# peaceminusones/Group-GAN-GCN-GAT

Measured on AMD Instinct MI355X. Metric: scenes/sec (obs8/pred12, 20 peds) at 1/2/4/8 GPUs; ADE/FDE vs ref, higher is better.
Workload: dtype fp32; 1 GPU; train iteration = D-step + G-step (best_k=20, Adam), GAT generator; BASELINE configs[1] shape (batch 64); scenes_per_gpu=64, global_batch=64, obs_len=8, pred_len=12, generator=gat, hip_graph=True, parallelism=dp1

## Files before the change

### group-gan-gcn-gat_amd/csrc/head.hip

```cpp
#include "sgg_common.h"

namespace sgg {

namespace {

constexpr int kHeadRows = 64;

__device__ __forceinline__ float bce_grad(float x, float y) {
  const float e = expf(-fabsf(x));
  const float sg = x > 0.f ? 1.f : (x < 0.f ? -1.f : 0.f);
  return (x >= 0.f ? 1.f : 0.f) - y - sg * (e / (1.f + e));
}

template <int NT, int KT>
__global__ void __launch_bounds__(256) head_fwd_kernel(const float* __restrict__ X, int ldx, int M,
                                                       const float* __restrict__ W1, const float* __restrict__ b1,
                                                       const float* __restrict__ w2, const float* __restrict__ b2,
                                                       int act, float* __restrict__ hid, float* __restrict__ Y) {
  constexpr int K = 16 * KT, KS = 4 * KT;
  const int lane = threadIdx.x & 63, wave = threadIdx.x >> 6;
  const int c16 = lane & 15, q = lane >> 4;
  const int row0 = blockIdx.x * kHeadRows + wave * 16;
  const float* xr = X + (size_t)min(row0 + c16, M - 1) * ldx;
  float a[KS], b[KS][NT], bc[NT], wc[NT];
#pragma unroll
  for (int m = 0; m < KT; ++m) {
    const float4 xv = *reinterpret_cast<const float4*>(xr + 16 * m + 4 * q);
    a[4 * m] = xv.x;
    a[4 * m + 1] = xv.y;
    a[4 * m + 2] = xv.z;
    a[4 * m + 3] = xv.w;
#pragma unroll
    for (int t = 0; t < NT; ++t) {
      const float4 wv = *reinterpret_cast<const float4*>(W1 + (size_t)(16 * t + c16) * K + 16 * m + 4 * q);
      b[4 * m][t] = wv.x;
      b[4 * m + 1][t] = wv.y;
      b[4 * m + 2][t] = wv.z;
      b[4 * m + 3][t] = wv.w;
    }
  }
#pragma unroll
  for (int t = 0; t < NT; ++t) {
    bc[t] = b1[16 * t + c16];
    wc[t] = w2[16 * t + c16];
  }
  const float bb2 = b2[0];
  floatx4 acc[NT];
#pragma unroll
  for (int t = 0; t < NT; ++t) acc[t] = floatx4{0.f, 0.f, 0.f, 0.f};
#pragma unroll
  for (int s = 0; s < KS; ++s)
#pragma unroll
    for (int t = 0; t < NT; ++t) acc[t] = __builtin_amdgcn_mfma_f32_16x16x4f32(a[s], b[s][t], acc[t], 0, 0, 0);
  const int N1 = 16 * NT;
  float p[4] = {0.f, 0.f, 0.f, 0.f};
#pragma unroll
  for (int t = 0; t < NT; ++t)
#pragma unroll
    for (int r = 0; r < 4; ++r) {
      float h = acc[t][r] + bc[t];
      if (act & 1) h = h > 0.f ? h : 0.f;
      const int m = row0 + 4 * q + r;
      if (m < M) hid[(size_t)m * N1 + 16 * t + c16] = h;
      p[r] = fmaf(h, wc[t], p[r]);
    }
#pragma unroll
  for (int r = 0; r < 4; ++r) {
#pragma unroll
    for (int o = 1; o < 16; o <<= 1) p[r] += __shfl_xor(p[r], o);
    float y = p[r] + bb2;
    if (act & 2) y = y > 0.f ? y : 0.f;
    const int m = row0 + 4 * q + r;
    if (c16 == 0 && m < M) Y[m] = y;
  }
}

template <int NT, int KT, int DP>
__device__ __forceinline__ void head_bwd_tail(const float* __restrict__ X, int ldx, int M, int rb,
                                              const float (&dh)[kHeadRows][DP], const float (&hg)[kHeadRows][DP],
                                              const float (&g2s)[kHeadRows], const float (&wb)[4 * NT][KT],
                                              float* __restrict__ dX, int lddx, float* __restrict__ wslab) {
  constexpr int N1 = 16 * NT, K = 16 * KT;
  const int tid = threadIdx.x;
  const int lane = tid & 63, wave = tid >> 6;
  const int c16 = lane & 15, q = lane >> 4;
  {
    floatx4 acc[KT];
#pragma unroll
    for (int t = 0; t < KT; ++t) acc[t] = floatx4{0.f, 0.f, 0.f, 0.f};
#pragma unroll
    for (int s = 0; s < N1 / 4; ++s) {
      const float a = dh[16 * wave + c16][4 * s + q];
#pragma unroll
      for (int t = 0; t < KT; ++t) acc[t] = __builtin_amdgcn_mfma_f32_16x16x4f32(a, wb[s][t], acc[t], 0, 0, 0);
    }
#pragma unroll
    for (int t = 0; t < KT; ++t)
#pragma unroll
      for (int r = 0; r < 4; ++r) {
        const int m = rb + 16 * wave + 4 * q + r;
        if (m < M) dX[(size_t)m * lddx + 16 * t + c16] = acc[t][r];
      }
  }
  if (!wslab) return;
  float* row = wslab + (size_t)blockIdx.x * (N1 * K + 2 * N1 + 1);
  for (int tile = wave; tile < NT * KT; tile += 4) {
    const int mt = tile / KT, nt = tile - mt * KT;
    floatx4 acc = floatx4{0.f, 0.f, 0.f, 0.f};
    float xb[kHeadRows / 4];
#pragma unroll
    for (int s = 0; s < kHeadRows / 4; ++s)
      xb[s] = X[(size_t)min(rb + 4 * s + q, M - 1) * ldx + 16 * nt + c16];
#pragma unroll
    for (int s = 0; s < kHeadRows / 4; ++s) {
      const float a = dh[4 * s + q][16 * mt + c16];
      acc = __builtin_amdgcn_mfma_f32_16x16x4f32(a, xb[s], acc, 0, 0, 0);
    }
#pragma unroll
    for (int r = 0; r < 4; ++r) row[(size_t)(16 * mt + 4 * q + r) * K + 16 * nt + c16] = acc[r];
  }
  for (int n = tid; n < N1; n += 256) {
    float s1 = 0.f, s2 = 0.f;
    for (int r = 0; r < kHeadRows; ++r) {
      s1 += dh[r][n];
      s2 += hg[r][n];
    }
    row[N1 * K + n] = s1;
    row[N1 * K + N1 + n] = s2;
  }
  if (tid == 0) {
    float s = 0.f;
    for (int r = 0; r < kHeadRows; ++r) s += g2s[r];
    row[N1 * K + 2 * N1] = s;
  }
}

__device__ __forceinline__ float bce_dy(float y, int m, int M, float gw, float ya, float yb, int split, int nv) {
  const bool first = m < split;
  const float cnt = first ? (float)min(split, nv) : (float)min(M - split, nv);
  const bool live = first ? m < nv : m - split < nv;
  return live ? (gw / cnt) * bce_grad(y, first ? ya : yb) : 0.f;
}

template <int NT, int KT>
__global__ void __launch_bounds__(256) head_bwd_kernel(const float* __restrict__ X, int ldx, int M,
                                                       const float* __restrict__ W1, const float* __restrict__ w2,
                                                       const float* __restrict__ hid, const float* __restrict__ Y,
                                                       const float* __restrict__ dY, int act,
                                                       float* __restrict__ dX, int lddx, float* __restrict__ wslab,
                                                       const float* __restrict__ bce_g, const float* __restrict__ bce_ya,
                                                       const float* __restrict__ bce_yb, int bce_split, float bce_w,
                                                       const int32_t* __restrict__ bce_nvalid) {
  constexpr int N1 = 16 * NT, K = 16 * KT;
  constexpr int DP = N1 + 4;
  __shared__ float dh[kHeadRows][DP];
  __shared__ float hg[kHeadRows][DP];
  __shared__ float g2s[kHeadRows];
  const int tid = threadIdx.x;
  const int lane = tid & 63;
  const int c16 = lane & 15, q = lane >> 4;
  const int rb = blockIdx.x * kHeadRows;
  float wb[N1 / 4][KT];
#pragma unroll
  for (int s = 0; s < N1 / 4; ++s)
#pragma unroll
    for (int t = 0; t < KT; ++t) wb[s][t] = W1[(size_t)(4 * s + q) * K + 16 * t + c16];
  {
    constexpr int RPT = kHeadRows * N1 / 256;
    constexpr int RS = 256 / N1;
    const int n = tid % N1, r0 = tid / N1;
    const float wn = w2[n];
    float hv[RPT], yv[RPT], dyv[RPT];
#pragma unroll
    for (int i = 0; i < RPT; ++i) {
      const int mc = min(rb + r0 + RS * i, M - 1);
      hv[i] = hid[(size_t)mc * N1 + n];
      yv[i] = Y[mc];
      dyv[i] = bce_g ? 0.f : dY[mc];
    }
    if (bce_g) {
      const float gw = *bce_g * bce_w, ya = *bce_ya, yb = *bce_yb;
      const int nv = bce_nvalid ? *bce_nvalid : M;
#pragma unroll
      for (int i = 0; i < RPT; ++i) {
        const int mc = min(rb + r0 + RS * i, M - 1);
        dyv[i] = bce_dy(yv[i], mc, M, gw, ya, yb, bce_split, nv);
      }
    }
#pragma unroll
    for (int i = 0; i < RPT; ++i) {
      const int r = r0 + RS * i, m = rb + r;
      const float g = (m < M && (!(act & 2) || yv[i] > 0.f)) ? dyv[i] : 0.f;
      dh[r][n] = (!(act & 1) || hv[i] > 0.f) ? g * wn : 0.f;
      hg[r][n] = g * hv[i];
      if (n == 0) g2s[r] = g;
    }
  }
  __syncthreads();
  head_bwd_tail<NT, KT, DP>(X, ldx, M, rb, dh, hg, g2s, wb, dX, lddx, wslab);
}

template <int NT, int KT>
__global__ void __launch_bounds__(256) head_fwdbwd_kernel(
    const float* __restrict__ X, int ldx, int M, const float* __restrict__ W1, const float* __restrict__ b1,
    const float* __restrict__ w2, const float* __restrict__ b2, int act, float* __restrict__ Y,
    float* __restrict__ dX, int lddx, float* __restrict__ wslab, const float* __restrict__ bce_g,
    const float* __restrict__ bce_ya, const float* __restrict__ bce_yb, int bce_split, float bce_w,
    const int32_t* __restrict__ bce_nvalid) {
  constexpr int N1 = 16 * NT, K = 16 * KT, KS = 4 * KT;
  constexpr int DP = N1 + 4;
  __shared__ float dh[kHeadRows][DP];
  __shared__ float hg[kHeadRows][DP];
  __shared__ float g2s[kHeadRows];
  const int lane = threadIdx.x & 63, wave = threadIdx.x >> 6;
  const int c16 = lane & 15, q = lane >> 4;
  const int rb = blockIdx.x * kHeadRows;
  const int row0 = rb + wave * 16;
  const float* xr = X + (size_t)min(row0 + c16, M - 1) * ldx;
  float a[KS], b[KS][NT], bc[NT], wc[NT];
#pragma unroll
  for (int m = 0; m < KT; ++m) {
    const float4 xv = *reinterpret_cast<const float4*>(xr + 16 * m + 4 * q);
    a[4 * m] = xv.x;
    a[4 * m + 1] = xv.y;
    a[4 * m + 2] = xv.z;
    a[4 * m + 3] = xv.w;
#pragma unroll
    for (int t = 0; t < NT; ++t) {
      const float4 wv = *reinterpret_cast<const float4*>(W1 + (size_t)(16 * t + c16) * K + 16 * m + 4 * q);
      b[4 * m][t] = wv.x;
      b[4 * m + 1][t] = wv.y;
      b[4 * m + 2][t] = wv.z;
      b[4 * m + 3][t] = wv.w;
    }
  }
  float wb[N1 / 4][KT];
#pragma unroll
  for (int s = 0; s < N1 / 4; ++s)
#pragma unroll
    for (int t = 0; t < KT; ++t) wb[s][t] = W1[(size_t)(4 * s + q) * K + 16 * t + c16];
#pragma unroll
  for (int t = 0; t < NT; ++t) {
    bc[t] = b1[16 * t + c16];
    wc[t] = w2[16 * t + c16];
  }
  const float bb2 = b2[0];
  const float gw = *bce_g * bce_w, ya = *bce_ya, yb = *bce_yb;
  const int nv = bce_nvalid ? *bce_nvalid : M;
  floatx4 acc[NT];
#pragma unroll
  for (int t = 0; t < NT; ++t) acc[t] = floatx4{0.f, 0.f, 0.f, 0.f};
#pragma unroll
  for (int s = 0; s < KS; ++s)
#pragma unroll
    for (int t = 0; t < NT; ++t) acc[t] = __builtin_amdgcn_mfma_f32_16x16x4f32(a[s], b[s][t], acc[t], 0, 0, 0);
  float h[NT][4];
  float p[4] = {0.f, 0.f, 0.f, 0.f};
#pragma unroll
  for (int t = 0; t < NT; ++t)
#pragma unroll
    for (int r = 0; r < 4; ++r) {
      float v = acc[t][r] + bc[t];
      if (act & 1) v = v > 0.f ? v : 0.f;
      h[t][r] = v;
      p[r] = fmaf(v, wc[t], p[r]);
    }
#pragma unroll
  for (int r = 0; r < 4; ++r) {
#pragma unroll
    for (int o = 1; o < 16; o <<= 1) p[r] += __shfl_xor(p[r], o);
    float y = p[r] + bb2;
    if (act & 2) y = y > 0.f ? y : 0.f;
    const int lr = wave * 16 + 4 * q + r, m = rb + lr;
    if (c16 == 0 && m < M) Y[m] = y;
    const float dy = bce_dy(y, min(m, M - 1), M, gw, ya, yb, bce_split, nv);
    const float g = (m < M && (!(act & 2) || y > 0.f)) ? dy : 0.f;
#pragma unroll
    for (int t = 0; t < NT; ++t) {
      const int n = 16 * t + c16;
      dh[lr][n] = (!(act & 1) || h[t][r] > 0.f) ? g * wc[t] : 0.f;
      hg[lr][n] = g * h[t][r];
    }
    if (c16 == 0) g2s[lr] = g;
  }
  __syncthreads();
  head_bwd_tail<NT, KT, DP>(X, ldx, M, rb, dh, hg, g2s, wb, dX, lddx, wslab);
}

template <int NT>
int launch_fwd_nt(const float* X, int ldx, int M, int K, const float* W1, const float* b1, const float* w2,
                  const float* b2, int act, float* hid, float* Y, hipStream_t st) {
  const dim3 grid((M + kHeadRows - 1) / kHeadRows);
  switch (K) {
    case 16: hipLaunchKernelGGL((head_fwd_kernel<NT, 1>), grid, dim3(256), 0, st, X, ldx, M, W1, b1, w2, b2, act, hid, Y); break;
// ... 122 lines not shown
```

### group-gan-gcn-gat_amd/csrc/pool.hip

```cpp
#include <stdlib.h>
#include <string.h>

#include "sgg_common.h"
#include "pool_common.h"

namespace sgg {


constexpr int kKT = 64;
constexpr int kKTP = kKT + 2;
constexpr int kPoolWaves = 4;

struct PoolSet {
  const float* U;
  const float* pos;
  const int32_t* scene_off;
  const int4* chunks;
  int nchunks;
  const int32_t* nchunks_dev;
  float* out;
  int32_t* argmax;
};

#define SGG_POOL_PICK(s1, s2, g1)                                                       \
  const bool two_ = (int)blockIdx.x >= (g1);                                            \
  const float* __restrict__ U = two_ ? s2.U : s1.U;                                     \
  const float* __restrict__ pos = two_ ? s2.pos : s1.pos;                               \
  const int32_t* __restrict__ scene_off = two_ ? s2.scene_off : s1.scene_off;           \
  const int4* __restrict__ chunks = two_ ? s2.chunks : s1.chunks;                       \
  float* __restrict__ out = two_ ? s2.out : s1.out;                                     \
  int32_t* __restrict__ argmax = two_ ? s2.argmax : s1.argmax;                          \
  const int32_t* ncd_ = two_ ? s2.nchunks_dev : s1.nchunks_dev;                         \
  const int nch = ncd_ ? *ncd_ : (two_ ? s2.nchunks : s1.nchunks);                      \
  const int gb_ = (int)blockIdx.x - (two_ ? (g1) : 0);                                  \
  const int gstride = two_ ? (int)gridDim.x - (g1) : (g1);                              \
  const int xb = (gb_ & 7) * (gstride >> 3) + (gb_ >> 3)

template <int BN, int GPW, int UNR>
__global__ void __launch_bounds__(256)
__attribute__((amdgpu_waves_per_eu(BN == 8 && GPW == 1 ? 5 : 1))) pool_fwd_kernel(
    const PoolSet s1, const PoolSet s2, int g1, const float* __restrict__ A,
    const float* __restrict__ W2 , const float* __restrict__ b2) {
  using C = PoolCfg<BN>;
  constexpr int NT = C::NT, BNP = C::BNP;
  extern __shared__ __attribute__((aligned(16))) char smem[];
  float* Us = reinterpret_cast<float*>(smem);
  float* W2s = Us + SGG_POOL_MAX_PEDS * kKTP;
  float* As = W2s + kKT * BNP;
  float2* ps = reinterpret_cast<float2*>(As + 2 * kKT);
  unsigned long long* keys = reinterpret_cast<unsigned long long*>(ps + SGG_POOL_MAX_PEDS);
  const int lane = threadIdx.x & 63;
  const int wave = __builtin_amdgcn_readfirstlane(threadIdx.x >> 6);
  const int c16 = lane & 15, kq = lane >> 4;
  float bv[NT];
#pragma unroll
  for (int t = 0; t < NT; ++t) bv[t] = b2[min(16 * t + c16, BN - 1)];

  SGG_POOL_PICK(s1, s2, g1);
  for (int ch = xb; ch < nch; ch += gstride) {
    const int4 cd = chunks[ch];
    const int s = cd.x, i0 = cd.y, i1 = cd.z;
    if (i1 <= i0) continue;
    const int o = scene_off[s];
    const int n = scene_off[s + 1] - o;
    const int rows = i1 - i0;
    const int npairs = rows * n;

    for (int q = threadIdx.x; q < n; q += blockDim.x) ps[q] = make_float2(pos[2 * (o + q)], pos[2 * (o + q) + 1]);
    for (int q = threadIdx.x; q < rows * BN; q += blockDim.x) keys[q] = 0ull;
    __syncthreads();

    int uoff[GPW];
    float rx[GPW], ry[GPW];
    floatx4 acc[GPW][NT];
#pragma unroll
    for (int g = 0; g < GPW; ++g) {
      const int p = (wave * GPW + g) * 16 + c16;
      int il = 0, j = 0;
      if (p < npairs) { il = p / n; j = p - il * n; }
      uoff[g] = j * kKTP + kq;
      const float2 pj = ps[j], pi = ps[i0 + il];
      rx[g] = p < npairs ? pj.x - pi.x : 0.f;
      ry[g] = p < npairs ? pj.y - pi.y : 0.f;
#pragma unroll
      for (int t = 0; t < NT; ++t) acc[g][t] = floatx4{0.f, 0.f, 0.f, 0.f};
    }

    constexpr int kUQ = (SGG_POOL_MAX_PEDS * (kKT / 4) + 255) / 256;
    constexpr int kWQ = (kKT * BNP + 255) / 256;
    float4 ureg[kUQ];
    float wreg[kWQ];
    float areg = 0.f;
    auto load_tile = [&](int k0) {
#pragma unroll
      for (int e = 0; e < kUQ; ++e) {
        const int q = threadIdx.x + 256 * e;
        const int r = q / (kKT / 4), c4 = q - r * (kKT / 4);
        if (r < n) ureg[e] = *reinterpret_cast<const float4*>(U + (size_t)(o + r) * kHidden + k0 + 4 * c4);
      }
#pragma unroll
      for (int e = 0; e < kWQ; ++e) {
        const int q = threadIdx.x + 256 * e;
        const int kk = q / BNP, cc = q - kk * BNP;
        wreg[e] = (kk < kKT && cc < BN) ? W2[(size_t)cc * kHidden + k0 + kk] : 0.f;
      }
      if (threadIdx.x < 2 * kKT) areg = A[2 * k0 + threadIdx.x];
    };
    auto store_tile = [&]() {
#pragma unroll
      for (int e = 0; e < kUQ; ++e) {
        const int q = threadIdx.x + 256 * e;
        const int r = q / (kKT / 4), c4 = q - r * (kKT / 4);
        if (r < n) {
          float* d = Us + r * kKTP + 4 * c4;
          d[0] = ureg[e].x; d[1] = ureg[e].y; d[2] = ureg[e].z; d[3] = ureg[e].w;
        }
      }
#pragma unroll
      for (int e = 0; e < kWQ; ++e) {
        const int q = threadIdx.x + 256 * e;
        if (q < kKT * BNP) W2s[q] = wreg[e];
      }
      if (threadIdx.x < 2 * kKT) As[threadIdx.x] = areg;
    };
    load_tile(0);
    __syncthreads();
    store_tile();
    __syncthreads();
    for (int k0 = 0; k0 < kHidden; k0 += kKT) {
      if (k0 + kKT < kHidden) load_tile(k0 + kKT);
      float b[NT], u[GPW];
      float2 a;
#pragma unroll
      for (int t = 0; t < NT; ++t) b[t] = W2s[kq * BNP + 16 * t + c16];
      a = *reinterpret_cast<const float2*>(As + 2 * kq);
#pragma unroll
      for (int g = 0; g < GPW; ++g) u[g] = Us[uoff[g]];
#pragma unroll UNR
      for (int s4 = 0; s4 < kKT / 4; ++s4) {
        float h[GPW], bc[NT];
#pragma unroll
        for (int g = 0; g < GPW; ++g) h[g] = fmaxf(fmaf(a.y, ry[g], fmaf(a.x, rx[g], u[g])), 0.f);
#pragma unroll
        for (int t = 0; t < NT; ++t) bc[t] = b[t];
        if (s4 + 1 < kKT / 4) {
          const int kn = 4 * (s4 + 1);
#pragma unroll
          for (int t = 0; t < NT; ++t) b[t] = W2s[(kn + kq) * BNP + 16 * t + c16];
          a = *reinterpret_cast<const float2*>(As + 2 * (kn + kq));
#pragma unroll
          for (int g = 0; g < GPW; ++g) u[g] = Us[uoff[g] + kn];
        }
#pragma unroll
        for (int g = 0; g < GPW; ++g)
#pragma unroll
          for (int t = 0; t < NT; ++t) acc[g][t] = __builtin_amdgcn_mfma_f32_16x16x4f32(h[g], bc[t], acc[g][t], 0, 0, 0);
      }
// ... 681 lines not shown
    const int c = q / (kHidden / 4), c4 = q - c * (kHidden / 4);
    float4 w = make_float4(0.f, 0.f, 0.f, 0.f);
    if (c < BN) w = *reinterpret_cast<const float4*>(W2 + (size_t)c * kHidden + 4 * c4);
    __bf16* d = W2s + c * kBfWP + 4 * c4;
    d[0] = (__bf16)w.x;
    d[1] = (__bf16)w.y;
    d[2] = (__bf16)w.z;
    d[3] = (__bf16)w.w;
  }
  for (int q = tid; q < kHidden; q += kBfThreads) {
    const float2 a = reinterpret_cast<const float2*>(A)[q];
    As[q] = a.x;
    As[kHidden + q] = a.y;
  }

  SGG_POOL_PICK(s1, s2, g1);
  for (int ch = xb; ch < nch; ch += gstride) {
    const int4 cd = chunks[ch];
    const int s = cd.x;
    if (cd.z <= cd.y) continue;
    const int o = scene_off[s];
    const int n = scene_off[s + 1] - o;
    const int i0 = cd.y, R = min(cd.z - cd.y, kBfMaxRows);
    const int nj = (n + kJbRows - 1) / kJbRows;
    __syncthreads();
    for (int q = tid; q < n; q += kBfThreads) ps[q] = make_float2(pos[2 * (o + q)], pos[2 * (o + q) + 1]);
    for (int q = tid; q < R * BN; q += kBfThreads) keys[q] = 0ull;

    floatx4 ur[kJbUQ];
    auto load_block = [&](int jb) __attribute__((always_inline)) {
#pragma unroll
      for (int e = 0; e < kJbUQ; ++e) {
        const int q = tid + kBfThreads * e;
        const int row = q / (kHidden / 4), c4 = q - row * (kHidden / 4);
        const int j = jb * kJbRows + row;
        ur[e] = j < n ? *reinterpret_cast<const floatx4*>(U + (size_t)(o + j) * kHidden + 4 * c4)
                      : floatx4{0.f, 0.f, 0.f, 0.f};
      }
    };
    auto store_block = [&](int buf) __attribute__((always_inline)) {
      float* d = Uj + buf * kJbRows * kJbUP;
#pragma unroll
      for (int e = 0; e < kJbUQ; ++e) {
        const int q = tid + kBfThreads * e;
        const int row = q / (kHidden / 4), c4 = q - row * (kHidden / 4);
        *reinterpret_cast<floatx4*>(d + row * kJbUP + 4 * c4) = ur[e];
      }
    };
    load_block(0);
    store_block(0);
    if (nj > 1) load_block(1);
    __syncthreads();

    for (int jb = 0; jb < nj; ++jb) {
      const float* ut = Uj + (jb & 1) * kJbRows * kJbUP;
      const int j = jb * kJbRows + c16;
      const bool jok = j < n;
      const float2 pj = ps[jok ? j : 0];
      for (int r0 = 0; r0 < R; r0 += kBfWaves * GPW) {
        float2v rxy[GPW];
        floatx4 acc[GPW][NT];
#pragma unroll
        for (int g = 0; g < GPW; ++g) {
          const int il = r0 + wave * GPW + g;
          const float2 pi = ps[i0 + min(il, R - 1)];
          rxy[g] = jok ? float2v{pj.x - pi.x, pj.y - pi.y} : float2v{0.f, 0.f};
#pragma unroll
          for (int t = 0; t < NT; ++t) acc[g][t] = floatx4{0.f, 0.f, 0.f, 0.f};
        }
        const int ngr = min(GPW, max(0, R - r0 - wave * GPW));
        const float* urow = ut + c16 * kJbUP + 8 * kq;
#pragma unroll 2
        for (int ks = 0; ks < kHidden / 32; ++ks) {
          const int ku = 32 * ks + 8 * kq;
          float2v ax[4], ay[4];
#pragma unroll
          for (int v = 0; v < 2; ++v) {
            const float4 x = *reinterpret_cast<const float4*>(As + ku + 4 * v);
            const float4 y = *reinterpret_cast<const float4*>(As + kHidden + ku + 4 * v);
            ax[2 * v] = float2v{x.x, x.y};
            ax[2 * v + 1] = float2v{x.z, x.w};
            ay[2 * v] = float2v{y.x, y.y};
            ay[2 * v + 1] = float2v{y.z, y.w};
          }
          bf16x8_t bfr[NT];
#pragma unroll
          for (int t = 0; t < NT; ++t)
            bfr[t] = *reinterpret_cast<const bf16x8_t*>(W2s + (16 * t + c16) * kBfWP + ku);
          const float4 u0 = *reinterpret_cast<const float4*>(urow + 32 * ks);
          const float4 u1 = *reinterpret_cast<const float4*>(urow + 32 * ks + 4);
          const float2v uv[4] = {{u0.x, u0.y}, {u0.z, u0.w}, {u1.x, u1.y}, {u1.z, u1.w}};
#pragma unroll
          for (int g = 0; g < GPW; ++g) {
            if (g < ngr) {
              const float2v rx2 = rxy[g].xx, ry2 = rxy[g].yy;
              short2v hi[4];
#pragma unroll
              for (int m = 0; m < 4; ++m) {
                const float2v pre = __builtin_elementwise_fma(ay[m], ry2, __builtin_elementwise_fma(ax[m], rx2, uv[m]));
                const short2v b = __builtin_bit_cast(short2v, __builtin_convertvector(pre, bf16x2v));
                hi[m] = __builtin_elementwise_max(b, short2v{0, 0});
              }
              const short4v h01 = __builtin_shufflevector(hi[0], hi[1], 0, 1, 2, 3);
              const short4v h23 = __builtin_shufflevector(hi[2], hi[3], 0, 1, 2, 3);
              const bf16x8_t hv =
                  __builtin_bit_cast(bf16x8_t, __builtin_shufflevector(h01, h23, 0, 1, 2, 3, 4, 5, 6, 7));
#pragma unroll
              for (int t = 0; t < NT; ++t)
                acc[g][t] = __builtin_amdgcn_mfma_f32_16x16x32_bf16(hv, bfr[t], acc[g][t], 0, 0, 0);
            }
          }
        }
#pragma unroll
        for (int g = 0; g < GPW; ++g) {
          if (g < ngr) {
            const int il = r0 + wave * GPW + g;
#pragma unroll
            for (int t = 0; t < NT; ++t) {
              const int cc = 16 * t + c16;
              const float bb = cc < BN ? bv[t] : 0.f;
              unsigned long long best = 0ull;
#pragma unroll
              for (int r = 0; r < 4; ++r) {
                const int jj = jb * kJbRows + 4 * kq + r;
                float v = acc[g][t][r] + bb;
                v = v > 0.f ? v : 0.f;
                const unsigned long long key =
                    jj < n ? (((unsigned long long)__float_as_uint(v) << 32) | (0xFFFFFFFFull - (unsigned)jj)) : 0ull;
                best = umax64(best, key);
              }
              best = rows_max64(best);
              if (kq == 0 && cc < BN) atomicMax(&keys[il * BN + cc], best);
            }
          }
        }
      }
      if (jb + 1 < nj) {
        store_block((jb + 1) & 1);
        if (jb + 2 < nj) load_block(jb + 2);
      }
      __syncthreads();
    }
    for (int q = tid; q < R * BN; q += kBfThreads) {
      const unsigned long long key = keys[q];
      const size_t oi = (size_t)(o + i0) * BN + q;
      out[oi] = __uint_as_float((unsigned)(key >> 32));
      argmax[oi] = o + (int)(0xFFFFFFFFu - (unsigned)(key & 0xFFFFFFFFull));
    }
  }
}

constexpr int kBwdStageRows = 16;

template <int BN, bool WGRAD, bool STAGE>
__global__ void __launch_bounds__(512) pool_bwd_kernel(
    const float* __restrict__ U, const float* __restrict__ pos, const float* __restrict__ A,
    const float* __restrict__ W2 , const float* __restrict__ out,
    const int32_t* __restrict__ argmax, const float* __restrict__ dout, const int32_t* __restrict__ scene_off,
    int S, int jq, float* __restrict__ dU, float* __restrict__ part) {
  __shared__ unsigned long long msk[SGG_POOL_MAX_PEDS * BN];
  __shared__ float gs[SGG_POOL_MAX_PEDS * BN];
  __shared__ int jsel[SGG_POOL_MAX_PEDS * BN];
  __shared__ float2 ps[SGG_POOL_MAX_PEDS];
  extern __shared__ float Us[];
  const int k = threadIdx.x;
  float w2[BN], dw2[BN];
#pragma unroll
  for (int c = 0; c < BN; ++c) {
    w2[c] = W2[c * kHidden + k];
    dw2[c] = 0.f;
  }
  const float a0 = A[2 * k], a1 = A[2 * k + 1];
  float dA0 = 0.f, dA1 = 0.f, db2 = 0.f;
  for (int un = blockIdx.x; un < S * jq; un += gridDim.x) {
    const int s = un / jq, jp = un - s * jq;
    const int o = scene_off[s];
    const int n = scene_off[s + 1] - o;
    const int ne = n * BN;
    const int j0 = (n * jp) / jq, j1 = (n * (jp + 1)) / jq;
    if (STAGE) {
      const float* Ur = U + (size_t)(o + j0) * kHidden + k;
#pragma unroll 4
      for (int r = 0; r < j1 - j0; ++r) Us[r * kHidden + k] = Ur[(size_t)r * kHidden];
    }
#pragma unroll 2
    for (int e = k; e < ne; e += kHidden) {
      const size_t ge = (size_t)o * BN + e;
      const float ov = out[ge], dv = dout[ge];
      const int av = argmax[ge];
      gs[e] = ov > 0.f ? dv : 0.f;
      jsel[e] = av - o;
      msk[e] = 0ull;
    }
    for (int q = k; q < n; q += kHidden) ps[q] = make_float2(pos[2 * (o + q)], pos[2 * (o + q) + 1]);
    __syncthreads();
    for (int e = k; e < ne; e += kHidden) {
      if (gs[e] != 0.f) {
        const int i = e / BN, c = e - i * BN;
        atomicOr(&msk[jsel[e] * BN + c], 1ull << i);
      }
    }
    if (WGRAD && jp == 0 && k < BN)
      for (int i = 0; i < n; ++i) db2 += gs[i * BN + k];
    __syncthreads();
    const float* Uc = U + (size_t)o * kHidden + k;
    float u_next = STAGE ? 0.f : (j0 < j1 ? Uc[(size_t)j0 * kHidden] : 0.f);
    for (int j = j0; j < j1; ++j) {
      float u;
      if (STAGE) {
        u = Us[(j - j0) * kHidden + k];
      } else {
        u = u_next;
        if (j + 1 < j1) u_next = Uc[(size_t)(j + 1) * kHidden];
      }
      const float2 pj = ps[j];
      float du = 0.f;
      constexpr int CB = BN < 16 ? BN : 16;
      unsigned long long mrow[CB];
#pragma unroll
      for (int c = 0; c < BN; ++c) {
        if (c % CB == 0) {
#pragma unroll
          for (int cc = 0; cc < CB; ++cc) mrow[cc] = msk[j * BN + c + cc];
        }
        const unsigned long long mv = mrow[c % CB];
        const unsigned mhi = (unsigned)__builtin_amdgcn_readfirstlane((unsigned)(mv >> 32));
        const unsigned mlo = (unsigned)__builtin_amdgcn_readfirstlane((unsigned)mv);
        unsigned long long m = ((unsigned long long)mhi << 32) | (unsigned long long)mlo;
        auto entry = [&](float g, float2 pi) {
          const float rx = pj.x - pi.x, ry = pj.y - pi.y;
          const float pre = fmaf(a1, ry, fmaf(a0, rx, u));
          const float gm = pre > 0.f ? g : 0.f;
          const float d = gm * w2[c];
          du += d;
          if (WGRAD) {
            dw2[c] = fmaf(gm, pre, dw2[c]);
            dA0 = fmaf(d, rx, dA0);
            dA1 = fmaf(d, ry, dA1);
          }
        };
        while (m) {
          const int i = __builtin_ctzll(m);
          m &= m - 1;
          const bool two = m != 0;
          const int i2 = two ? __builtin_ctzll(m) : i;
          if (two) m &= m - 1;
          const float g = gs[i * BN + c], g2 = gs[i2 * BN + c];
          const float2 pi = ps[i], pi2 = ps[i2];
          entry(g, pi);
          if (two) entry(g2, pi2);
        }
      }
      dU[(size_t)(o + j) * kHidden + k] = du;
    }
    __syncthreads();
  }
  if (WGRAD) {
    float* row = part + (size_t)blockIdx.x * (BN * kHidden + 2 * kHidden + BN);
#pragma unroll
    for (int c = 0; c < BN; ++c) row[c * kHidden + k] = dw2[c];
    row[BN * kHidden + 2 * k] = dA0;
    row[BN * kHidden + 2 * k + 1] = dA1;
    if (k < BN) row[BN * kHidden + 2 * kHidden + k] = db2;
  }
}

template <int BN>
static size_t pool_fwd_lds(int max_rows) {
  using C = PoolCfg<BN>;
  return sizeof(float) * ((size_t)SGG_POOL_MAX_PEDS * kKTP + (size_t)kKT * C::BNP + 2 * kKT) +
         sizeof(float2) * SGG_POOL_MAX_PEDS + sizeof(unsigned long long) * (size_t)max_rows * BN;
}

static int pool_range(int nchunks) { return nchunks < 32768 ? (nchunks + 7) & ~7 : 32768; }

template <int BN, int GPW>
static void launch_fwd_g(const PoolSet& s1, const PoolSet& s2, const float* A, const float* W2, const float* b2,
                         int max_rows, int max_n, hipStream_t st) {
  const int g1 = pool_range(s1.nchunks), grid = g1 + (s2.chunks ? pool_range(s2.nchunks) : 0);
  const int nchunks = s1.nchunks + (s2.chunks ? s2.nchunks : 0);
  const size_t lds = pool_fwd_lds<BN>(max_rows);
  if constexpr (GPW <= 2 && BN >= 32 && BN <= 48) {
    const char* xe = getenv("SGG_POOL_X3");
    if (!(xe && xe[0] == '0') && max_n >= 1 && max_n <= SGG_POOL_MAX_PEDS) {
      const int umax = (max_n + 3) & ~3;
      const size_t lx = sizeof(float) * 2 * ((size_t)umax * kVP + pool_x3_tb_fixed<BN>()) +
                        sizeof(float2) * SGG_POOL_MAX_PEDS + sizeof(unsigned long long) * (size_t)max_rows * BN;
      hipLaunchKernelGGL((pool_fwd_x3_kernel<BN, GPW>), dim3(grid), dim3(256), lx, st, s1, s2, g1, A, W2, b2, umax);
      return;
    }
  }
  if constexpr (GPW <= 2) {
    const char* vv = getenv("SGG_POOL_V");
    if (nchunks <= 4 * device_cus() && !(vv && vv[0] == '0')) {
      const size_t lv = sizeof(float) * 2 * ((size_t)(SGG_POOL_MAX_PEDS + 16 * PoolCfg<BN>::NT) * kVP + 2 * kKT) +
                        sizeof(float2) * SGG_POOL_MAX_PEDS + sizeof(unsigned long long) * (size_t)max_rows * BN;
      hipLaunchKernelGGL((pool_fwd_v_kernel<BN, GPW>), dim3(grid), dim3(256), lv, st, s1, s2, g1, A, W2, b2);
      return;
    }
  }
  hipLaunchKernelGGL((pool_fwd_kernel<BN, GPW, 2>), dim3(grid), dim3(256), lds, st, s1, s2, g1, A, W2, b2);
}
static int pool_bwd_jq(int S) {
  if (S < 1) return 1;
  const int jq = 256 / S;
  return jq < 1 ? 1 : (jq > 8 ? 8 : jq);
}

template <int BN>
static int launch_fwd(const PoolSet& s1, const PoolSet& s2, const float* A, const float* W2, const float* b2,
                      int max_rows, int max_n, int gpw, hipStream_t st) {
  switch (gpw) {
    case 1: launch_fwd_g<BN, 1>(s1, s2, A, W2, b2, max_rows, max_n, st); break;
    case 2: launch_fwd_g<BN, 2>(s1, s2, A, W2, b2, max_rows, max_n, st); break;
    default: launch_fwd_g<BN, 4>(s1, s2, A, W2, b2, max_rows, max_n, st); break;
  }
  SGG_RETURN_LAUNCH("sgg_pool_fwd");
}

template <int BN>
static int launch_fwd_bf16(const PoolSet& s1, const PoolSet& s2, const float* A, const float* W2, const float* b2,
                           int gpw, int max_rows, int max_n, hipStream_t st) {
  const int n1 = s1.nchunks, n2 = s2.chunks ? s2.nchunks : 0;
  int grid = device_cus();
  if (grid > n1 + n2) grid = n1 + n2;
  grid = (grid + 7) & ~7;
  int g1 = grid;
  if (n2 > 0) {
    if (n1 == 0) {
      g1 = 0;
    } else {
      if (grid < 16) grid = 16;
      g1 = (int)(((long long)grid * n1 / (n1 + n2) + 4) & ~7LL);
      g1 = g1 < 8 ? 8 : (g1 > grid - 8 ? grid - 8 : g1);
    }
  }
  const char* jbe = getenv("SGG_POOL_JB");
  const bool jb_off = jbe && strcmp(jbe, "0") == 0;
  if (max_n >= 32 && !jb_off && pool_jb_lds_bytes<BN>() <= 160 * 1024) {
    const size_t ljb = pool_jb_lds_bytes<BN>();
#define SGG_POOL_JB(G) \
  hipLaunchKernelGGL((pool_fwd_bf16_jb_kernel<BN, G>), dim3(grid), dim3(kBfThreads), ljb, st, s1, s2, g1, A, W2, b2)
    if (max_rows > 16)
      SGG_POOL_JB(4);
    else if (max_rows > 8)
      SGG_POOL_JB(2);
    else
      SGG_POOL_JB(1);
#undef SGG_POOL_JB
    SGG_RETURN_LAUNCH("sgg_pool_fwd_bf16");
  }
  const size_t lds = pool_bf16_lds_bytes<BN>();
#define SGG_POOL_BF(G) \
  hipLaunchKernelGGL((pool_fwd_bf16_kernel<BN, G>), dim3(grid), dim3(kBfThreads), lds, st, s1, s2, g1, A, W2, b2)
  if (gpw >= 4 && BN <= 48)
    SGG_POOL_BF(4);
  else if (gpw >= 2)
    SGG_POOL_BF(2);
  else
    SGG_POOL_BF(1);
#undef SGG_POOL_BF
  SGG_RETURN_LAUNCH("sgg_pool_fwd_bf16");
}

template <int BN>
static int launch_bwd(const float* U, const float* pos, const float* A, const float* W2, const float* out,
                      const int32_t* am, const float* dout, const int32_t* off, int S, int max_n, float* dU,
                      float* part, hipStream_t st) {
  const int grid = sgg_pool_bwd_grid(S), jq = pool_bwd_jq(S);
  const int rows = (max_n + jq - 1) / jq + 1;
  const bool stage = rows <= kBwdStageRows;
  const size_t lds = stage ? sizeof(float) * (size_t)rows * kHidden : 0;
#define SGG_POOL_BWD(W, SG)                                                                                          \
  hipLaunchKernelGGL((pool_bwd_kernel<BN, W, SG>), dim3(grid), dim3(512), lds, st, U, pos, A, W2, out, am, dout, off, \
                     S, jq, dU, part)
  if (part) {
    if (stage) SGG_POOL_BWD(true, true); else SGG_POOL_BWD(true, false);
  } else {
    if (stage) SGG_POOL_BWD(false, true); else SGG_POOL_BWD(false, false);
  }
#undef SGG_POOL_BWD
  SGG_RETURN_LAUNCH("sgg_pool_bwd");
}

}

using namespace sgg;

static bool pool_bn_ok(int bn) { return bn == 8 || bn == 16 || bn == 32 || bn == 48 || bn == 64; }

static int plan_rows(int n, int gpw) {
  int rows = (16 * kPoolWaves * gpw) / n;
  if (rows > 64) rows = 64;
  return rows < 1 ? 1 : rows;
}

extern "C" int sgg_pool_plan(const int32_t* host_scene_off, int S, int bn, int target_chunks, int max_gpw,
                             int32_t* chunks, int cap, int* max_rows, int* gpw_out) {
  if (!host_scene_off || !chunks || !max_rows || !gpw_out || S < 0 || cap < 0) {
    sgg::set_error("sgg_pool_plan: bad argument");
    return SGG_E_ARG;
  }
  int gpw = bn > 16 ? 4 : 2;
  if (max_gpw > 0) {
    while (gpw > max_gpw && gpw > 1) gpw >>= 1;
  }
  for (; gpw > 1; gpw >>= 1) {
    long nc = 0;
    for (int s = 0; s < S; ++s) {
      const int n = host_scene_off[s + 1] - host_scene_off[s];
      if (n > 0) nc += (n + plan_rows(n, gpw) - 1) / plan_rows(n, gpw);
    }
    if (nc >= target_chunks) break;
  }
  int nc = 0, mr = 1;
  for (int s = 0; s < S; ++s) {
    const int n = host_scene_off[s + 1] - host_scene_off[s];
    if (n <= 0) continue;
    const int rmax = plan_rows(n, gpw), nck = (n + rmax - 1) / rmax, rows = (n + nck - 1) / nck;
    for (int i0 = 0; i0 < n; i0 += rows) {
      const int i1 = i0 + rows < n ? i0 + rows : n;
      if (nc >= cap) {
        sgg::set_error("sgg_pool_plan: chunk table capacity %d exceeded", cap);
        return SGG_E_ARG;
      }
      chunks[4 * nc + 0] = s;
      chunks[4 * nc + 1] = i0;
      chunks[4 * nc + 2] = i1;
      chunks[4 * nc + 3] = gpw;
      if (i1 - i0 > mr) mr = i1 - i0;
      ++nc;
    }
  }
  *max_rows = mr;
  *gpw_out = gpw;
  return nc;
}

extern "C" int sgg_pool_plan_bf16(const int32_t* host_scene_off, int S, int bn, int target_chunks, int32_t* chunks,
                                  int cap, int* max_rows, int* gpw_out) {
  if (!host_scene_off || !chunks || !max_rows || !gpw_out || S < 0 || cap < 0 || !pool_bn_ok(bn)) {
    sgg::set_error("sgg_pool_plan_bf16: bad argument");
    return SGG_E_ARG;
  }
  auto rows_of = [&](int n, int pb) { const int r = pb / n; return r < 1 ? 1 : (r > n ? n : r); };
  int pb = 2048;
  for (; pb > 128; pb >>= 1) {
    long nc = 0;
    for (int s = 0; s < S; ++s) {
      const int n = host_scene_off[s + 1] - host_scene_off[s];
      if (n > 0) nc += (n + rows_of(n, pb) - 1) / rows_of(n, pb);
    }
    if (nc >= target_chunks) break;
  }
  int nc = 0, mr = 1, mp = 1;
  for (int s = 0; s < S; ++s) {
    const int n = host_scene_off[s + 1] - host_scene_off[s];
    if (n <= 0) continue;
    const int rmax = rows_of(n, pb), nck = (n + rmax - 1) / rmax, rows = (n + nck - 1) / nck;
    for (int i0 = 0; i0 < n; i0 += rows) {
      const int i1 = i0 + rows < n ? i0 + rows : n;
      if (nc >= cap) {
        sgg::set_error("sgg_pool_plan_bf16: chunk table capacity %d exceeded", cap);
        return SGG_E_ARG;
      }
      chunks[4 * nc + 0] = s;
      chunks[4 * nc + 1] = i0;
      chunks[4 * nc + 2] = i1;
      chunks[4 * nc + 3] = 0;
      if (i1 - i0 > mr) mr = i1 - i0;
      if ((i1 - i0) * n > mp) mp = (i1 - i0) * n;
      ++nc;
    }
  }
  const int gmax = bn > 48 ? 2 : 4;
  int gpw = 1;
  while (gpw < gmax && 16 * kBfWaves * gpw < mp) gpw <<= 1;
  for (int c = 0; c < nc; ++c) chunks[4 * c + 3] = gpw;
  *max_rows = mr;
  *gpw_out = gpw;
  return nc;
}

static int pool_batch_check(const char* fn, const float* U, const float* pos, const int32_t* scene_off,
                            const int32_t* chunks, int nchunks, int max_rows, int gpw, int B, int max_n,
                            const float* out, const int32_t* argmax) {
  SGG_CHECK_ARG(U && pos && scene_off && chunks && out && argmax, "%s: null pointer", fn);
  SGG_CHECK_ARG(nchunks >= 0 && B >= 0, "%s: bad sizes", fn);
  SGG_CHECK_ARG(max_n >= 1 && max_n <= SGG_POOL_MAX_PEDS, "%s: max scene size %d outside [1, %d]", fn, max_n,
                SGG_POOL_MAX_PEDS);
  SGG_CHECK_ARG(max_rows >= 1 && max_rows <= 64, "%s: chunk rows %d outside [1, 64]", fn, max_rows);
  SGG_CHECK_ARG(gpw == 1 || gpw == 2 || gpw == 4, "%s: gpw %d not in {1,2,4}", fn, gpw);
  return 0;
}

static int pool_fwd_sets(const PoolSet& s1, const PoolSet& s2, const float* A, const float* W2, const float* b2,
                         int max_rows, int max_n, int gpw, int bn, bool bf16, hipStream_t st) {
  if (s1.nchunks + (s2.chunks ? s2.nchunks : 0) == 0) return 0;
  if (bf16) {
    switch (bn) {
      case 8: return launch_fwd_bf16<8>(s1, s2, A, W2, b2, gpw, max_rows, max_n, st);
      case 16: return launch_fwd_bf16<16>(s1, s2, A, W2, b2, gpw, max_rows, max_n, st);
      case 32: return launch_fwd_bf16<32>(s1, s2, A, W2, b2, gpw, max_rows, max_n, st);
      case 48: return launch_fwd_bf16<48>(s1, s2, A, W2, b2, gpw, max_rows, max_n, st);
      default: return launch_fwd_bf16<64>(s1, s2, A, W2, b2, gpw, max_rows, max_n, st);
    }
  }
  switch (bn) {
    case 8: return launch_fwd<8>(s1, s2, A, W2, b2, max_rows, max_n, gpw, st);
    case 16: return launch_fwd<16>(s1, s2, A, W2, b2, max_rows, max_n, gpw, st);
    case 32: return launch_fwd<32>(s1, s2, A, W2, b2, max_rows, max_n, gpw, st);
    case 48: return launch_fwd<48>(s1, s2, A, W2, b2, max_rows, max_n, gpw, st);
    default: return launch_fwd<64>(s1, s2, A, W2, b2, max_rows, max_n, gpw, st);
  }
}

static int pool_fwd_one(const char* fn, bool bf16, const float* U, const float* pos, const float* A, const float* W2,
                        const float* b2, const int32_t* scene_off, const int32_t* chunks, int nchunks, int max_rows,
                        int gpw, int B, int bn, int max_n, float* out, int32_t* argmax, const int32_t* nchunks_dev,
                        void* stream) {
  SGG_CHECK_ARG(A && W2 && b2, "%s: null pointer", fn);
  SGG_CHECK_ARG(pool_bn_ok(bn), "%s: bottleneck %d not built (8/16/32/48/64)", fn, bn);
  const int rc = pool_batch_check(fn, U, pos, scene_off, chunks, nchunks, max_rows, gpw, B, max_n, out, argmax);
  if (rc != 0) return rc;
  const PoolSet s1 = {U, pos, scene_off, reinterpret_cast<const int4*>(chunks), nchunks, nchunks_dev, out, argmax};
  const PoolSet none = {};
  return pool_fwd_sets(s1, none, A, W2, b2, max_rows, max_n, gpw, bn, bf16, (hipStream_t)stream);
}

extern "C" int sgg_pool_fwd(const float* U, const float* pos, const float* A, const float* W2, const float* b2,
                            const int32_t* scene_off, const int32_t* chunks, int nchunks, int max_rows, int gpw,
                            int B, int bn, int max_n, float* out, int32_t* argmax, const int32_t* nchunks_dev,
                            void* stream) {
  return pool_fwd_one("sgg_pool_fwd", false, U, pos, A, W2, b2, scene_off, chunks, nchunks, max_rows, gpw, B, bn,
                      max_n, out, argmax, nchunks_dev, stream);
}

extern "C" int sgg_pool_fwd_bf16(const float* U, const float* pos, const float* A, const float* W2, const float* b2,
                                 const int32_t* scene_off, const int32_t* chunks, int nchunks, int max_rows, int gpw,
                                 int B, int bn, int max_n, float* out, int32_t* argmax, const int32_t* nchunks_dev,
                                 void* stream) {
  return pool_fwd_one("sgg_pool_fwd_bf16", true, U, pos, A, W2, b2, scene_off, chunks, nchunks, max_rows, gpw, B,
                      bn, max_n, out, argmax, nchunks_dev, stream);
}

extern "C" int sgg_pool_fwd2(const SggPoolBatch* a, const SggPoolBatch* b, const float* A, const float* W2,
                             const float* b2, int bn, int bf16, void* stream) {
  SGG_CHECK_ARG(a && b && A && W2 && b2, "sgg_pool_fwd2: null pointer");
  SGG_CHECK_ARG(pool_bn_ok(bn), "sgg_pool_fwd2: bottleneck %d not built (8/16/32/48/64)", bn);
  for (const SggPoolBatch* p : {a, b}) {
    const int rc = pool_batch_check("sgg_pool_fwd2", p->U, p->pos, p->scene_off, p->chunks, p->nchunks, p->max_rows,
                                    p->gpw, p->B, p->max_n, p->out, p->argmax);
    if (rc != 0) return rc;
  }
  SGG_CHECK_ARG(a->gpw == b->gpw, "sgg_pool_fwd2: the batches' plans differ in gpw (%d, %d)", a->gpw, b->gpw);
  const PoolSet s1 = {a->U, a->pos, a->scene_off, reinterpret_cast<const int4*>(a->chunks), a->nchunks,
                      a->nchunks_dev, a->out, a->argmax};
  const PoolSet s2 = {b->U, b->pos, b->scene_off, reinterpret_cast<const int4*>(b->chunks), b->nchunks,
                      b->nchunks_dev, b->out, b->argmax};
  const int mr = a->max_rows > b->max_rows ? a->max_rows : b->max_rows;
  const int mn = a->max_n > b->max_n ? a->max_n : b->max_n;
  return pool_fwd_sets(s1, s2, A, W2, b2, mr, mn, a->gpw, bn, bf16 != 0, (hipStream_t)stream);
}

extern "C" int sgg_pool_bwd_grid(int S) {
  if (S < 1) return 1;
  const long long u = (long long)S * pool_bwd_jq(S);
  return (int)(u < 256 ? u : 256);
}

extern "C" int sgg_pool_bwd(const float* U, const float* pos, const float* A, const float* W2, const float* out,
                            const int32_t* argmax, const float* dout, const int32_t* scene_off, int S, int B,
                            int bn, int max_n, float* dU, float* part, void* stream) {
  SGG_CHECK_ARG(U && pos && A && W2 && out && argmax && dout && scene_off && dU, "sgg_pool_bwd: null pointer");
  SGG_CHECK_ARG(pool_bn_ok(bn), "sgg_pool_bwd: bottleneck %d not built", bn);
  SGG_CHECK_ARG(max_n >= 1 && max_n <= SGG_POOL_MAX_PEDS, "sgg_pool_bwd: max scene size %d outside [1, %d]",
                max_n, SGG_POOL_MAX_PEDS);
  SGG_CHECK_ARG(S >= 0 && B >= 0, "sgg_pool_bwd: bad sizes");
  hipStream_t st = (hipStream_t)stream;
  if (S == 0) return 0;
  switch (bn) {
    case 8: return launch_bwd<8>(U, pos, A, W2, out, argmax, dout, scene_off, S, max_n, dU, part, st);
    case 16: return launch_bwd<16>(U, pos, A, W2, out, argmax, dout, scene_off, S, max_n, dU, part, st);
    case 32: return launch_bwd<32>(U, pos, A, W2, out, argmax, dout, scene_off, S, max_n, dU, part, st);
    case 48: return launch_bwd<48>(U, pos, A, W2, out, argmax, dout, scene_off, S, max_n, dU, part, st);
    default: return launch_bwd<64>(U, pos, A, W2, out, argmax, dout, scene_off, S, max_n, dU, part, st);
  }
}
```

### group-gan-gcn-gat_amd/sgan/_native.py

```python
import ctypes
import os

import torch

from ._srchash import source_hash

_LIB_EXPLICIT = bool(os.environ.get("SGG_LIB"))
_LIB_PATH = os.environ.get("SGG_LIB") or os.path.join(os.path.dirname(os.path.abspath(__file__)), "_lib", "libsgg.so")

_i = ctypes.c_int
_f = ctypes.c_float
_p = ctypes.c_void_p
_sz = ctypes.c_size_t

MAX_HEADS = 4


class GatEncWeights(ctypes.Structure):
    _fields_ = [("Wi", _p * MAX_HEADS), ("ai", _p * MAX_HEADS), ("Wio", _p), ("aio", _p),
                ("Wg", _p * MAX_HEADS), ("ag", _p * MAX_HEADS), ("Wgo", _p), ("ago", _p), ("Woe", _p), ("boe", _p)]


class GatEncArgs(ctypes.Structure):
    _fields_ = [("X", _p), ("ldx", _i), ("labels", _p), ("scene_off", _p), ("S", _i), ("np", _i), ("nh", _i),
                ("alpha", _f), ("w", GatEncWeights), ("y", _p), ("ldy", _i), ("dy", _p), ("lddy", _i), ("dX", _p),
                ("lddx", _i), ("slab", _p), ("saved", _p), ("X2", _p), ("ldx2", _i), ("kx1", _i),
                ("dX2", _p), ("lddx2", _i), ("dy_copies", _i), ("dy_cstride", _i)]


_pargs = ctypes.POINTER(GatEncArgs)


class GcnModArgs(ctypes.Structure):
    _fields_ = [("X", _p), ("ldx", _i), ("X2", _p), ("ldx2", _i), ("kx1", _i), ("labels", _p), ("scene_off", _p),
                ("S", _i), ("np", _i), ("fin", _i), ("fe", _i), ("bf16", _i), ("W0i", _p), ("W1i", _p), ("W0g", _p),
                ("W1g", _p), ("Woe", _p), ("boe", _p), ("y", _p), ("ldy", _i), ("dy", _p), ("lddy", _i),
                ("dy_copies", _i), ("dy_cstride", _i), ("dX", _p), ("lddx", _i), ("dX2", _p), ("lddx2", _i),
                ("slab", _p)]


_gargs = ctypes.POINTER(GcnModArgs)


class LstmSeg(ctypes.Structure):
    _fields_ = [("rel", _p), ("A", _p), ("Whh", _p), ("bias", _p), ("h0", _p), ("c0", _p), ("T", _i), ("B", _i),
                ("Bl", _i), ("t0", _i), ("Tl", _i), ("Bsrc", _i), ("h_all", _p), ("c_all", _p), ("act_all", _p),
                ("Wu", _p), ("ldwu", _i), ("cu", _p), ("NU", _i), ("U", _p)]


_sargs = ctypes.POINTER(LstmSeg)


class PoolDh(ctypes.Structure):
    _fields_ = [("dU", _p), ("ldu", _i), ("W1h", _p), ("ldw", _i), ("base", _p), ("NU", _i), ("h", _p), ("ldh", _i),
                ("ws", _p), ("ws_bytes", _sz), ("splits", _i)]


GLUE_NONE, GLUE_SELECT, GLUE_L2BWD = 0, 1, 2


class GlueSeg(ctypes.Structure):
    _fields_ = [("kind", _i), ("pred", _p), ("ldp", _i), ("gt", _p), ("mask", _p), ("ldm", _i), ("scene_off", _p),
                ("S", _i), ("T", _i), ("B", _i), ("k", _i), ("best", _p), ("w", _f), ("gout", _p), ("dpred", _p),
                ("ldd", _i), ("term", _p)]

FOLD_MAX = 8


class Fold(ctypes.Structure):
    _fields_ = [("W", _p), ("ldw", _i), ("R", _i), ("E", _i), ("We", _p), ("be", _p), ("b1", _p), ("b2", _p),
                ("A", _p), ("bias", _p)]

RED_MAX = 24
FOLDB_MAX = 6


class Red(ctypes.Structure):
    _fields_ = [("src", _p), ("rows", _i), ("ld", _i), ("col0", _i), ("cols", _i), ("out", _p), ("map", _i),
                ("N", _i), ("ldo", _i), ("trans", _i)]


class FoldBwd(ctypes.Structure):
    _fields_ = [("W", _p), ("ldw", _i), ("R", _i), ("E", _i), ("We", _p), ("be", _p),
                ("dA_src", _p), ("dA_rows", _i), ("dA_ld", _i), ("dA_col0", _i),
                ("db_src", _p), ("db_rows", _i), ("db_ld", _i), ("db_col0", _i),
                ("dW", _p), ("lddw", _i), ("dWe", _p), ("dbe", _p), ("dbias_copy", _p)]


class DecInit(ctypes.Structure):
    _fields_ = [("ctx", _p), ("ldc", _i), ("Dc", _i), ("z", _p), ("nz", _i), ("best", _p), ("first_k", _i),
                ("ped_scene", _p), ("S", _i), ("Bper", _i), ("last_rel", _p)]


LOSSJOB_MAX = 2


class TrajOut(ctypes.Structure):
    _fields_ = [("out", _p), ("NB", _i), ("T0", _i), ("col0", _i), ("ncol", _i), ("head", _p), ("ldh", _i),
                ("b", _p), ("ldb", _i), ("pos0", _p), ("start", _p)]


class PoolBatch(ctypes.Structure):
    _fields_ = [("U", _p), ("pos", _p), ("scene_off", _p), ("chunks", _p), ("nchunks", _i), ("max_rows", _i),
                ("gpw", _i), ("B", _i), ("max_n", _i), ("out", _p), ("argmax", _p), ("nchunks_dev", _p)]


class GatLayerSet(ctypes.Structure):
    _fields_ = [("x1", _p), ("ld1", _i), ("K1", _i), ("x2", _p), ("ld2", _i), ("K2", _i), ("seg_off", _p),
                ("nseg", _i), ("n", _i), ("max_seg", _i), ("xn", _p), ("rstd", _p), ("wh", _p), ("hp", _p), ("y", _p),
                ("ldy", _i)]


class L2Job(ctypes.Structure):
    _fields_ = [("term", _p), ("S", _i), ("loss", _p)]


class BceJob(ctypes.Structure):
    _fields_ = [("x", _p), ("n", _i), ("split", _i), ("ya", _p), ("yb", _p), ("w", _f), ("loss", _p),
                ("addend", _p), ("total", _p), ("nvalid", _p)]


SIGNATURES = {
    "sgg_version": (_i, []),
    "sgg_last_error": (ctypes.c_char_p, []),
    "sgg_source_hash": (ctypes.c_char_p, []),
    "sgg_xw": (_i, [_p, _i, _p, _i, _p, _i, _i, _p, _p, _i, _i, _i, _i, _i, _p]),
    "sgg_xw_bf16": (_i, [_p, _i, _p, _i, _p, _i, _i, _p, _p, _i, _i, _i, _i, _i, _p]),
    "sgg_pool_plan": (_i, [_p, _i, _i, _i, _i, _p, _i, _p, _p]),
    "sgg_pool_fwd": (_i, [_p, _p, _p, _p, _p, _p, _p, _i, _i, _i, _i, _i, _i, _p, _p, _p, _p]),
    "sgg_pool_plan_bf16": (_i, [_p, _i, _i, _i, _p, _i, _p, _p]),
    "sgg_pool_fwd_bf16": (_i, [_p, _p, _p, _p, _p, _p, _p, _i, _i, _i, _i, _i, _i, _p, _p, _p, _p]),
    "sgg_pool_fwd2": (_i, [ctypes.POINTER(PoolBatch), ctypes.POINTER(PoolBatch), _p, _p, _p, _i, _i, _p]),
    "sgg_pool_bwd_grid": (_i, [_i]),
    "sgg_pool_dh_dw": (_i, [_p, _i, _p, _i, _p, _i, _i, _p, _i, _i, _i, _p, _sz, _p]),
    "sgg_pool_bwd": (_i, [_p, _p, _p, _p, _p, _p, _p, _p, _i, _i, _i, _i, _p, _p, _p]),
    "sgg_pool_plan_wide": (_i, [_p, _i, _i, _i, _p, _i, _p, _p]),
    "sgg_pool_fwd_wide": (_i, [_p, _p, _p, _p, _p, _p, _p, _i, _i, _i, _i, _i, _i, _p, _p, _p]),
    "sgg_pool_bwd_wide_grid": (_i, [_i, _i]),
    "sgg_pool_bwd_wide": (_i, [_p, _p, _p, _p, _p, _p, _p, _p, _i, _i, _i, _i, _p, _p, _p]),
    "sgg_gat_fwd": (_i, [_p, _i, _p, _p, _p, _p, _i, _i, _i, _f, _i, _i, _i, _p, _p, _i, _p]),
    "sgg_gat_bwd": (_i, [_p, _i, _p, _p, _p, _i, _i, _i, _f, _i, _i, _i, _p, _p, _p, _i, _p, _p, _p, _p]),
    "sgg_gat_fwd_ex": (_i, [_p, _i, _p, _p, _p, _p, _p, _i, _i, _i, _f, _i, _i, _i, _p, _p, _i, _p]),
    "sgg_gat_bwd_ex": (_i, [_p, _i, _p, _p, _p, _p, _i, _i, _i, _f, _i, _i, _i, _p, _p, _p, _i, _p, _p, _p, _p, _p,
                            _p]),
    "sgg_gat_bwd_ex_work_bytes": (_sz, [_i, _i, _i]),
    "sgg_gat_wide_work_floats": (_sz, [_i, _i, _i, _i, _i]),
    "sgg_gat_fwd_wide": (_i, [_p, _i, _p, _p, _i, _p, _p, _p, _i, _i, _i, _f, _i, _i, _i, _p, _p, _i, _p, _p]),
    "sgg_gat_bwd_wide": (_i, [_p, _i, _p, _p, _i, _p, _p, _i, _i, _i, _f, _i, _i, _i, _p, _p, _p, _i, _p, _p, _p, _p,
                              _p, _p, _p, _p]),
    "sgg_gat_layer_lds_bytes": (_sz, [_i, _i, _i]),
    "sgg_gat_layer_fwd": (_i, [_p, _i, _i, _p, _i, _i, _p, _p, _p, _p, _p, _i, _i, _i, _i, _f, _f, _i, _i, _i, _p, _p,
                               _p, _p, _p, _i, _p]),
    "sgg_gat_layer_fwd2": (_i, [ctypes.POINTER(GatLayerSet), ctypes.POINTER(GatLayerSet), _p, _p, _p, _p, _i, _i, _f,
                                _f, _i, _i, _p]),
    "sgg_seg_norm_fwd": (_i, [_p, _i, _i, _p, _i, _f, _p, _i, _p, _p]),
    "sgg_seg_norm_bwd": (_i, [_p, _i, _p, _i, _i, _p, _i, _p, _p, _i, _p]),
    "sgg_group_index_ws": (_sz, [_i, _i]),
    "sgg_group_index": (_i, [_p, _p, _i, _i, _i, _p, _p, _p, _p, _p, _p, _p]),
    "sgg_seg_reduce": (_i, [_p, _i, _i, _p, _p, _p, _p, _p, _i, _i, _p, _i, _p]),
    "sgg_seg_gather": (_i, [_p, _i, _i, _p, _p, _p, _i, _p, _i, _p]),
    "sgg_xtw_splits": (_i, [_i, _i, _i]),
    "sgg_lstm_bwd_split": (_i, [_p, _p, _p, _p, _p, _p, _p, _p, _p, _p, _i, _i, _i, _i, _p, _p, _p, _p, _p]),
    "sgg_lstm_bwd_tail": (_i, [_p, _p, _p, _p, _p, _p, _p, _i, _i, _i, _i, _p, _p]),
    "sgg_lstm_fwd_seg": (_i, [_sargs, _i, _p]),
    "sgg_lstm_fwd_seg_glue": (_i, [_sargs, _i, ctypes.POINTER(GlueSeg), _p]),
    "sgg_lstm_fwd_seg2": (_i, [_sargs, _i, _sargs, _i, _p]),
    "sgg_lstm_fwd_seg3": (_i, [_sargs, _i, _sargs, _i, _sargs, _i, _p]),
    "sgg_lstm_bwd_shared": (_i, [_p, _p, _p, _p, _p, _p, _p, _i, _i, _i, _i, _i, _p, _p, _p]),
    "sgg_lstm_bwd_pooldh_ok": (_i, [_i]),
    "sgg_lstm_bwd_pooldh_pays": (_i, [_i, _i]),
    "sgg_lstm_bwd_pooldh_rides": (_i, [_i, _i, _i]),
    "sgg_lstm_bwd_pooldh": (_i, [_p, _p, _p, _p, _p, _p, ctypes.POINTER(PoolDh), _i, _i, _i, _i, _i, _i, _p, _p, _p,
                                 _p]),
    "sgg_lstm_u_ok": (_i, [_i, _i, _i, _i, _i, _i]),
    "sgg_lstm_fwd_u": (_i, [_p, _p, _p, _p, _p, _p, _i, _i, _i, _p, _p, _p, _p, _i, _p, _i, _p, _p]),
    "sgg_head_ok": (_i, [_i, _i]),
    "sgg_head_slab_cols": (_i, [_i, _i]),
    "sgg_head_fwd": (_i, [_p, _i, _i, _i, _i, _p, _p, _p, _p, _i, _p, _p, _p]),
    "sgg_head_bwd": (_i, [_p, _i, _i, _i, _i, _p, _p, _p, _p, _p, _i, _p, _i, _p, _p, _p, _p, _i, _f, _p, _p]),
    "sgg_head_fwdbwd": (_i, [_p, _i, _i, _i, _i, _p, _p, _p, _p, _i, _p, _p, _i, _p, _p, _p, _p, _i, _f, _p, _p]),
    "sgg_xtw_partial": (_i, [_p, _i, _p, _i, _p, _i, _i, _i, _i, _i, _p, _sz, _p]),
    "sgg_grad_finish": (_i, [ctypes.POINTER(Red), _i, ctypes.POINTER(FoldBwd), _i, _p, _sz, _p]),
    "sgg_lstm_fwd_dec": (_i, [ctypes.POINTER(DecInit), _p, _p, _p, _p, _p, _i, _i, _i, _p, _p, _p, _p, _p,
                              ctypes.POINTER(TrajOut), _p]),
    "sgg_lstm_fwd_dec2": (_i, [ctypes.POINTER(DecInit), ctypes.POINTER(DecInit), _p, _p, _p, _p, _p, _i, _i, _i, _i,
                               _p, _p, ctypes.POINTER(TrajOut), _p]),
    "sgg_lstm_fwd_dec_seg": (_i, [ctypes.POINTER(DecInit), _p, _p, _p, _p, _p, _i, _i, _i, _p, _p, _p, _p, _p,
                                  ctypes.POINTER(TrajOut), _sargs, _i, _p]),
    "sgg_grad_finish_losses": (_i, [ctypes.POINTER(Red), _i, ctypes.POINTER(FoldBwd), _i, _p, _sz,
                                    ctypes.POINTER(L2Job), _i, ctypes.POINTER(BceJob), _i, _p]),
    "sgg_adam_parts": (_i, [ctypes.c_longlong]),
    "sgg_adam_step": (_i, [_p, _p, _p, _p, _p, _i, ctypes.c_double, ctypes.c_double, ctypes.c_double, _f, _f, _p, _p,
                          _sz, _p]),
    "sgg_xtw": (_i, [_p, _i, _p, _i, _p, _i, _i, _i, _i, _p, _i, _i, _p, _p, _sz, _p]),
    "sgg_fold_fwd": (_i, [_p, _i, _i, _i, _p, _p, _p, _p, _p, _p, _p]),
    "sgg_fold_fwd_multi": (_i, [ctypes.POINTER(Fold), _i, _p]),
    "sgg_fold_bwd": (_i, [_p, _i, _i, _i, _p, _p, _p, _p, _p, _i, _p, _p, _p, _p]),
    "sgg_lstm_fwd": (_i, [_p, _p, _p, _p, _p, _p, _p, _p, _i, _i, _i, _i, _p, _p, _p, _p, _p]),
    "sgg_lstm_state_floats": (ctypes.c_longlong, [_i, _i, _i, _i]),
    "sgg_lstm_wpart_rows": (_i, [_i, _i]),
    "sgg_lstm_kernel_name": (ctypes.c_char_p, [_i, _i, _i, _i, _i]),
    "sgg_lstm_bwd": (_i, [_p, _p, _p, _p, _p, _p, _p, _p, _p, _p, _i, _i, _i, _i, _p, _p, _p, _p, _p, _p]),
    "sgg_bce_fwd": (_i, [_p, _i, _i, _p, _p, _f, _p, _p, _p, _p, _p]),
    "sgg_bce_bwd": (_i, [_p, _i, _i, _p, _p, _f, _p, _p, _p, _p]),
    "sgg_gatenc_param_size": (_i, [_i]),
    "sgg_gatenc_lds_bytes": (ctypes.c_longlong, [_i, _i, _i]),
    "sgg_gatenc_saved_floats": (ctypes.c_longlong, [_i, _i, _i]),
    "sgg_gatenc_fwd": (_i, [_pargs, _p]),
    "sgg_gatenc_fwd2": (_i, [_pargs, _pargs, _p]),
    "sgg_gatenc_bwd": (_i, [_pargs, _p]),
    "sgg_gcnmod_param_size": (_i, [_i, _i]),
    "sgg_gcnmod_slab_rows": (_i, [_i]),
    "sgg_gcnmod_lds_bytes": (ctypes.c_longlong, [_i, _i, _i, _i]),
    "sgg_gcnmod_fwd": (_i, [_gargs, _p]),
    "sgg_gcnmod_fwd2": (_i, [_gargs, _gargs, _p]),
    "sgg_gcnmod_bwd": (_i, [_gargs, _p]),
    "sgg_slab_reduce": (_i, [_p, _i, _i, _p, _p]),
    "sgg_gather_batch_floats": (ctypes.c_longlong, [_i, _i, _i]),
    "sgg_gather_batch": (_i, [_p, _i, _p, _i, _i, _i, _p, _p]),
    "sgg_traj_cat": (_i, [_p, _i, _i, _p, _i, _p, _i, _i, _i, _p, _p, _p, _p]),
    "sgg_decoder_init": (_i, [_p, _i, _i, _p, _i, _p, _i, _i, _p, _i, _i, _p, _p, _p, _p]),
    "sgg_l2_select": (_i, [_p, _p, _p, _i, _p, _i, _i, _i, _i, _p, _p]),
    "sgg_l2_loss_fwd": (_i, [_p, _i, _p, _p, _i, _p, _i, _i, _i, _f, _p, _p, _p, _p]),
    "sgg_l2_loss_bwd": (_i, [_p, _i, _p, _p, _i, _p, _p, _i, _i, _f, _p, _p, _i, _p]),
    "sgg_l2_loss_bwd_scenes": (_i, [_p, _i, _p, _p, _i, _p, _i, _i, _i, _f, _p, _p, _i, _p, _p]),
}

_lib = None


class NativeError(RuntimeError):
    pass


def lib_path():
    return _LIB_PATH


def built_hash():
    return load(require_gpu=False).sgg_source_hash().decode()


def load(require_gpu=True):
    global _lib
    if _lib is None:
        if not os.path.exists(_LIB_PATH):
            raise NativeError("libsgg.so not built at %s -- run group-gan-gcn-gat_amd/build_native.py "
                              "(or __graft_entry__.build())" % _LIB_PATH)
        lib = ctypes.CDLL(_LIB_PATH)
        for name, (res, args) in SIGNATURES.items():
            fn = getattr(lib, name)
            fn.restype = res
            fn.argtypes = args
        if not _LIB_EXPLICIT:
            built, tree = lib.sgg_source_hash().decode(), source_hash()
            if built != tree:
                raise NativeError("%s was built from other sources (hash %s) than this tree's csrc/ + "
                                  "include/sgg.h (%s) -- rebuild with group-gan-gcn-gat_amd/build_native.py"
                                  % (_LIB_PATH, built[:16], tree[:16]))
        _lib = lib
    if require_gpu and not torch.cuda.is_available():
        raise NativeError("sgan: no HIP device visible; the MI355X kernels have no CPU fallback")
    return _lib


def check(rc, name):
    if rc != 0:
        msg = _lib.sgg_last_error().decode(errors="replace")
        raise NativeError("%s failed (rc=%d): %s" % (name, rc, msg))


def stream_ptr():
    return ctypes.c_void_p(torch.cuda.current_stream().cuda_stream)


def ptr(t):
    if t is None:
        return None
    return ctypes.c_void_p(t.data_ptr())
```

### group-gan-gcn-gat_amd/sgan/kernels.py

```python
import contextlib
import functools
import os
import weakref

import torch

from . import _native as N

GATENC_FUSED = os.environ.get("SGG_GATENC_FUSED", "1") != "0"
GATENC_SAVE = os.environ.get("SGG_GATENC_SAVE", "1") != "0"
DUAL_POOL_BWD = os.environ.get("SGG_DUAL_POOL_BWD", "1") != "0"
POOL_DH_IN_LSTM = os.environ.get("SGG_POOL_DH_IN_LSTM", "1") != "0"


DEBUG = os.environ.get("SGG_DEBUG", "0") == "1"


def _lib():
    return N.load()


def _req(t, name, dtype=torch.float32):
    if not t.is_cuda:
        raise N.NativeError("%s must be a device tensor (no CPU path)" % name)
    if t.dtype != dtype:
        raise N.NativeError("%s must be %s, got %s" % (name, dtype, t.dtype))
    return t


def _rows(t, name):
    _req(t, name)
    if t.dim() != 2 or t.stride(1) != 1:
        t = t.contiguous()
    return t


@contextlib.contextmanager
def _scoped(slot, obj):
    prev = slot[0]
    slot[0] = obj
    try:
        yield obj
    finally:
        slot[0] = prev
        if hasattr(obj, "flush"):
            obj.flush()


_PRECISION = os.environ.get("SGG_PRECISION", "fp32")


def set_precision(p):
    global _PRECISION
    if p not in ("fp32", "bf16"):
        raise ValueError("precision must be 'fp32' or 'bf16'")
    _PRECISION = p


def precision():
    return _PRECISION


_private = {}
_hiprt = None


def private_stream(tag, device=None):
    global _hiprt
    import ctypes
    dev = torch.cuda.current_device() if device is None else torch.device(device).index
    if dev is None:
        dev = torch.cuda.current_device()
    key = (tag, dev)
    st = _private.get(key)
    if st is None:
        if _hiprt is None:
            lib = ctypes.CDLL(os.path.join(os.path.dirname(torch.__file__), "lib", "libamdhip64.so"))
            lib.hipStreamCreateWithFlags.argtypes = [ctypes.POINTER(ctypes.c_void_p), ctypes.c_uint]
            lib.hipStreamCreateWithFlags.restype = ctypes.c_int
            _hiprt = lib
        h = ctypes.c_void_p()
        with torch.cuda.device(dev):
            rc = _hiprt.hipStreamCreateWithFlags(ctypes.byref(h), 1)
        if rc != 0 or not h.value:
            raise N.NativeError("hipStreamCreateWithFlags failed (%d)" % rc)
        st = _private[key] = torch.cuda.ExternalStream(h.value, device=torch.device("cuda", dev))
    return st


def xw_raw(x, w, bias=None, trans_w=False, act=0, out=None, mask=None, prec=None):
    x = _rows(x, "x")
    if mask is not None:
        mask = _rows(mask, "mask")
        assert mask.shape == x.shape
    w = _rows(w, "w")
    M, K = x.shape
    Nn = w.shape[0] if trans_w else w.shape[1]
    assert (w.shape[1] if trans_w else w.shape[0]) == K, (x.shape, w.shape, trans_w)
    if bias is not None:
        bias = _req(bias, "bias").contiguous()
        assert bias.numel() == Nn
    y = out if out is not None else torch.empty(M, Nn, device=x.device, dtype=torch.float32)

    bf16 = (prec or _PRECISION) == "bf16"
    fn = _lib().sgg_xw_bf16 if bf16 else _lib().sgg_xw

    def launch():
        N.check(fn(N.ptr(x), x.stride(0), N.ptr(mask), mask.stride(0) if mask is not None else 0,
                   N.ptr(w), w.stride(0), int(bool(trans_w)), N.ptr(bias), N.ptr(y), y.stride(0), M, K, Nn,
                   int(act), N.stream_ptr()), "sgg_xw")
    launch()
    if timer.active and M > 0:
        tw = "true" if trans_w else "false"
        name = ("sgg::xw_bf16_kernel<%s>" % tw if bf16 else
                "sgg::xw_splitk_kernel<%s>" % tw if K >= 256 else
                "sgg::xw_kernel<true, true>" if trans_w and K <= 256 else
                "sgg::xw_kernel<%s, false>" % tw)
        timer.add(name, (M, K, Nn, mask is not None), 2.0 * M * K * Nn,
                  4.0 * (M * K * (2 if mask is not None else 1) + K * Nn + M * Nn), launch)
    return y


def xtw(X, Y, colsum=False, trans_c=False, out=None, mask=None):
    lib = _lib()
    X = _rows(X, "X")
    Y = _rows(Y, "Y")
    if mask is not None:
        mask = _rows(mask, "mask")
        assert mask.shape == Y.shape
    R, M = X.shape
    Nn = Y.shape[1]
    assert Y.shape[0] == R
    shape = (Nn, M) if trans_c else (M, Nn)
    if out is None:
        C = torch.empty(shape, device=X.device, dtype=torch.float32)
    else:
        assert tuple(out.shape) == shape and out.stride(1) == 1, (out.shape, shape)
        C = out
    if R == 0:
        C.zero_()
        return (C, torch.zeros(Nn, device=X.device)) if colsum else C
    splits = lib.sgg_xtw_splits(R, M, Nn)
    ws = torch.empty(splits * (M * Nn + Nn), device=X.device, dtype=torch.float32)
    cs = torch.empty(Nn, device=X.device, dtype=torch.float32) if colsum else None
    def launch():
        N.check(lib.sgg_xtw(N.ptr(X), X.stride(0), N.ptr(Y), Y.stride(0), N.ptr(mask),
                            mask.stride(0) if mask is not None else 0, R, M, Nn, N.ptr(C), C.stride(0), int(trans_c),
                            N.ptr(cs), N.ptr(ws), ws.numel() * 4, N.stream_ptr()), "sgg_xtw")
    launch()
    if timer.active:
        timer.add("sgg::xtw_partial_kernel+xtw_reduce_kernel", (R, M, Nn, mask is not None), 2.0 * R * M * Nn,
                  4.0 * (R * M + R * Nn * (2 if mask is not None else 1) + M * Nn) + 8.0 * ws.numel(), launch)
    return (C, cs) if colsum else C


def fold_fwd(W, We, be, b1, b2=None):
    key, ver = _fold_key(W, We, be, b1, b2)
    ent = _FOLD_CACHE.get(key)
    if _fold_hit(ent, ver, (W, We, be, b1, b2)):
        return ent[1], ent[2]
    prefold([(W, We, be, b1, b2)])
    ent = _FOLD_CACHE[key]
    return ent[1], ent[2]


# ... 149 lines not shown
DEFER_LOSSES = os.environ.get("SGG_DEFER_LOSSES", "1") != "0"


def _loss_deferrable(kind):
    return DEFER_LOSSES and _DEFER[0] > 0 and not _NO_DEFER[0] and len(_LOSS[kind]) < N.LOSSJOB_MAX


@contextlib.contextmanager
def eager_losses():
    prev = _NO_DEFER[0]
    _NO_DEFER[0] = True
    try:
        yield
    finally:
        _NO_DEFER[0] = prev


_NO_DEFER = [False]


def _queue_loss(kind, job, keep, outs):
    _LOSS[kind].append(job)
    _LOSS["keep"] += [t.untyped_storage() for t in keep if t is not None]
    _LOSS["out"].update(t.data_ptr() for t in outs)


def _loss_pending(t):
    return t is not None and t.data_ptr() in _LOSS["out"]


def _take_losses():
    glue_flush()
    l2, bce, keep = _LOSS["l2"], _LOSS["bce"], _LOSS["keep"]
    _LOSS.update(l2=[], bce=[], keep=[], out=set())
    return l2, bce, keep


def flush_losses():
    l2, bce, keep = _take_losses()
    if l2 or bce:
        _finish_launch([], [], keep, l2, bce)


@contextlib.contextmanager
def defer_grad_finish():
    if os.environ.get("SGG_CHECK_DEFER") == "1":
        yield
        return
    _DEFER[0] += 1
    try:
        yield
    finally:
        _DEFER[0] -= 1
        if _DEFER[0] == 0:
            grad_flush()


def grad_flush():
    if not _PENDING:
        flush_losses()
    while _PENDING:
        reds, folds, keep = [], [], []
        while _PENDING and len(reds) + len(_PENDING[0].reds) <= N.RED_MAX \
                and len(folds) + len(_PENDING[0].folds) <= N.FOLDB_MAX:
            gf = _PENDING.pop(0)
            reds += gf.reds
            folds += gf.folds
            keep += gf.keep
        if not reds and not folds:
            raise N.NativeError("grad_flush: a queued finish exceeds the job limits")
        l2, bce = [], []
        if not _PENDING:
            l2, bce, lkeep = _take_losses()
            keep = keep + lkeep
        _finish_launch(reds, folds, keep, l2, bce)


def _finish_launch(reds_l, folds_l, keep, l2_l=(), bce_l=()):
    lib = _lib()
    assert len(reds_l) <= N.RED_MAX and len(folds_l) <= N.FOLDB_MAX
    assert len(l2_l) <= N.LOSSJOB_MAX and len(bce_l) <= N.LOSSJOB_MAX
    reds = (N.Red * max(1, len(reds_l)))(*reds_l)
    folds = (N.FoldBwd * max(1, len(folds_l)))(*folds_l)
    l2 = (N.L2Job * max(1, len(l2_l)))(*l2_l)
    bce = (N.BceJob * max(1, len(bce_l)))(*bce_l)
    nr, nf, nl, nb = len(reds_l), len(folds_l), len(l2_l), len(bce_l)
    dev = keep[0].device
    scratch = torch.empty(max(1, sum(3 * f.R for f in folds_l)), device=dev, dtype=torch.float32)

    def launch(reds=reds, folds=folds, nr=nr, nf=nf, l2=l2, bce=bce, nl=nl, nb=nb, keep=list(keep)):
        N.check(lib.sgg_grad_finish_losses(reds, nr, folds, nf, N.ptr(scratch), scratch.numel() * 4, l2, nl, bce, nb,
                                           N.stream_ptr()), "sgg_grad_finish")
    launch()
    if timer.active:
        nb = sum(4.0 * r.rows * r.cols for r in reds_l) + sum(4.0 * 3 * f.R * max(f.dA_rows, f.db_rows)
                                                               for f in folds_l)
        timer.add("sgg::grad_finish_kernel", (nr, nf, tuple((r.rows, r.cols) for r in reds_l)), nb / 4.0, nb,
                  launch)


class _XW(torch.autograd.Function):
    @staticmethod
    def forward(ctx, x, w, bias, trans_w, act):
        y = xw_raw(x, w, bias, trans_w, act)
        ctx.trans_w, ctx.act, ctx.has_bias = trans_w, act, bias is not None
        ctx.save_for_backward(x, w, y if act else None)
        return y

    @staticmethod
    def backward(ctx, dy):
        x, w, y = ctx.saved_tensors
        dy = dy.contiguous()
        m = y if ctx.act else None
        dx = dw = db = None
        if ctx.needs_input_grad[0]:
            dx = xw_raw(dy, w, None, not ctx.trans_w, 0, mask=m, prec="fp32")
        if ctx.needs_input_grad[1] or (ctx.has_bias and ctx.needs_input_grad[2]):
            dw, cs = xtw(x, dy, colsum=True, trans_c=ctx.trans_w, mask=m)
            db = cs if ctx.has_bias else None
        return dx, dw, db, None, None


def xw(x, w, bias=None, trans_w=False, act=0):
    return _XW.apply(x, w, bias, trans_w, act)


def linear(x, lin, act=0):
    return _XW.apply(x, lin.weight, lin.bias, True, act)


def head_ok(seq):
    mods = list(seq)
    lins = [m for m in mods if isinstance(m, torch.nn.Linear)]
    if len(lins) != 2 or any(not isinstance(m, (torch.nn.Linear, torch.nn.ReLU)) for m in mods):
        return None
    l1, l2 = lins
    if l2.out_features != 1 or l1.bias is None or l2.bias is None:
        return None
    if not _lib().sgg_head_ok(l1.in_features, l1.out_features):
        return None
    i1, i2 = mods.index(l1), mods.index(l2)
    relu1 = i1 + 1 < len(mods) and isinstance(mods[i1 + 1], torch.nn.ReLU)
    relu2 = i2 + 1 < len(mods) and isinstance(mods[i2 + 1], torch.nn.ReLU)
    if len(mods) != 2 + int(relu1) + int(relu2):
        return None
    return l1, l2, int(relu1) | (2 * int(relu2))


class BceLink:

    def __init__(self):
        self.pending = None
        self.forward_held = None
        self.fused = None

    def put(self, g, ya, yb, split, w, placeholder, nvalid=None):
        self.pending = (g, ya, yb, split, w, placeholder, nvalid)

    def take(self):
        p, self.pending = self.pending, None
        return p

    def run_fused(self, ya, yb, split, w, nvalid):
        held, self.forward_held = self.forward_held, None
        if held is None:
            return
        x, W1, b1, W2, b2, act, y, wgrad = held
        lib = _lib()
        M, Kd = x.shape
        N1 = W1.shape[0]
        seed = const(1.0, x.device)
        dx = torch.empty(M, Kd, device=x.device, dtype=torch.float32)
        P = lib.sgg_head_slab_cols(Kd, N1)
        slab = torch.empty(max((M + 63) // 64, 1), P, device=x.device, dtype=torch.float32) if wgrad else None

        def launch():
            N.check(lib.sgg_head_fwdbwd(N.ptr(x), x.stride(0), M, Kd, N1, N.ptr(W1), N.ptr(b1), N.ptr(W2), N.ptr(b2),
                                        act, N.ptr(y), N.ptr(dx), dx.stride(0), N.ptr(slab), N.ptr(seed), N.ptr(ya),
                                        N.ptr(yb), int(split), float(w), N.ptr(nvalid), N.stream_ptr()),
                    "sgg_head_fwdbwd")
        launch()
        if timer.active and M > 0:
            timer.add("sgg::head_fwdbwd_kernel<%d, %d>" % (N1 // 16, Kd // 16), (M, Kd, N1, wgrad),
                      2.0 * M * N1 * (Kd + 1) + 2.0 * M * N1 * Kd * (2 if wgrad else 1),
                      4.0 * (M * Kd * (2 if wgrad else 1) + N1 * Kd + 2 * M + M * Kd
                             + (slab.numel() if wgrad else 0)), launch)
        self.fused = (seed, dx, slab)

    def flush_forward(self):
        held, self.forward_held = self.forward_held, None
        if held is not None:
            x, W1, b1, W2, b2, act, y, _ = held
            _head_fwd(x, W1, b1, W2, b2, act, y, record=True)


HEAD_FUSE = os.environ.get("SGG_HEAD_FUSE", "1") != "0"
_HELD_HEADS = []


def _head_fwd(x, W1, b1, W2, b2, act, y, record=False):
    lib = _lib()
    M, Kd = x.shape
    N1 = W1.shape[0]
    hid = torch.empty(M, N1, device=x.device, dtype=torch.float32)

    def launch():
        N.check(lib.sgg_head_fwd(N.ptr(x), x.stride(0), M, Kd, N1, N.ptr(W1), N.ptr(b1), N.ptr(W2), N.ptr(b2),
                                 act, N.ptr(hid), N.ptr(y), N.stream_ptr()), "sgg_head_fwd")
    launch()
    if record and timer.active and M > 0:
        timer.add("sgg::head_fwd_kernel<%d, %d>" % (N1 // 16, Kd // 16), (M, Kd, N1), 2.0 * M * N1 * (Kd + 1),
                  4.0 * (M * Kd + N1 * Kd + M * N1 + M), launch)
    return hid


class _Head(torch.autograd.Function):
    @staticmethod
    def forward(ctx, x, W1, b1, W2, b2, act, bce_link=None):
        x = _rows(x, "x")
        if x.data_ptr() % 16 or x.stride(0) % 4:
            x = x.contiguous()
        M, Kd = x.shape
        W1, W2 = W1.contiguous(), W2.contiguous()
        b1, b2 = b1.contiguous(), b2.contiguous()
        y = torch.empty(M, 1, device=x.device, dtype=torch.float32)
        wgrad = any(ctx.needs_input_grad[1:5])
        if bce_link is not None and HEAD_FUSE and M > 0:
            bce_link.forward_held = (x, W1, b1, W2, b2, act, y, wgrad)
            _HELD_HEADS.append(bce_link)
            hid = None
        else:
            hid = _head_fwd(x, W1, b1, W2, b2, act, y, record=True)
        ctx.act = act
        ctx.bce_link = bce_link
        ctx.hid = hid
        ctx.save_for_backward(x, W1, b1, W2, b2, y)
        return y

    @staticmethod
    def backward(ctx, dy):
        lib = _lib()
        x, W1, b1, W2, b2, y = ctx.saved_tensors
        need = ctx.needs_input_grad
        M, Kd = x.shape
        N1 = W1.shape[0]
        link = ctx.bce_link
        pend = link.take() if link is not None else None
        if link is not None and link.forward_held is not None:
            link.flush_forward()
        fused, hid = None, ctx.hid
        if link is not None and link.fused is not None:
            fused, link.fused = link.fused, None
        bce = None
        if pend is not None:
            g, ya, yb, split, w, ph, nvalid = pend
            if dy.data_ptr() != ph.data_ptr():
                raise N.NativeError("fused head + BCE backward: the scores have a consumer besides the BCE loss "
                                    "(set SGG_HEAD_BCE=0)")
            bce = (g.contiguous(), ya, yb, int(split), float(w), nvalid)
        else:
            dy = dy.contiguous()
        wgrad = any(need[1:5])
        P = lib.sgg_head_slab_cols(Kd, N1)
        rows = (M + 63) // 64
        if fused is not None and bce is not None and bce[0].data_ptr() == fused[0].data_ptr():
            dx, slab = fused[1], fused[2]
        else:
            if hid is None:
                hid = _head_fwd(x, W1, b1, W2, b2, ctx.act, torch.empty_like(y))
            dx = torch.empty(M, Kd, device=x.device, dtype=torch.float32)
            slab = torch.empty(max(rows, 1), P, device=x.device, dtype=torch.float32) if wgrad else None
            bg, bya, byb, bsp, bw, bnv = (N.ptr(bce[0]), N.ptr(bce[1]), N.ptr(bce[2]), bce[3], bce[4],
                                          N.ptr(bce[5])) if bce else (None, None, None, 0, 0.0, None)

            def launch():
                N.check(lib.sgg_head_bwd(N.ptr(x), x.stride(0), M, Kd, N1, N.ptr(W1), N.ptr(W2), N.ptr(hid),
                                         N.ptr(y), None if bce else N.ptr(dy), ctx.act, N.ptr(dx), dx.stride(0),
                                         N.ptr(slab), bg, bya, byb, bsp, bw, bnv, N.stream_ptr()), "sgg_head_bwd")
            launch()
            if timer.active and M > 0:
                timer.add("sgg::head_bwd_kernel<%d, %d>" % (N1 // 16, Kd // 16), (M, Kd, N1, wgrad),
                          2.0 * M * N1 * Kd * (2 if wgrad else 1),
                          4.0 * (M * Kd * (3 if wgrad else 2) + 2 * M * N1 + (slab.numel() if wgrad else 0)), launch)
        ctx.hid = None
        if not wgrad:
            return dx, None, None, None, None, None, None
        dW1 = torch.empty(N1, Kd, device=x.device, dtype=torch.float32)
        db1 = torch.empty(N1, device=x.device, dtype=torch.float32)
        dW2 = torch.empty(1, N1, device=x.device, dtype=torch.float32)
        db2 = torch.empty(1, device=x.device, dtype=torch.float32)
        if M == 0:
            for t in (dW1, db1, dW2, db2):
                t.zero_()
        else:
            gf = GradFinish()
            gf.rowsum(slab, rows, P, 0, N1 * Kd, dW1)
            gf.rowsum(slab, rows, P, N1 * Kd, N1, db1)
            gf.rowsum(slab, rows, P, N1 * Kd + N1, N1, dW2)
            gf.rowsum(slab, rows, P, N1 * Kd + 2 * N1, 1, db2)
            gf.run()
        return dx, dW1, db1, dW2, db2, None, None


HEAD_BCE = os.environ.get("SGG_HEAD_BCE", "1") != "0"
_BCE_HANDOFF = [0]


@contextlib.contextmanager
def bce_handoff():
    _BCE_HANDOFF[0] += 1
    try:
        yield
    finally:
        _BCE_HANDOFF[0] -= 1
        if _BCE_HANDOFF[0] == 0:
            while _HELD_HEADS:
                _HELD_HEADS.pop().flush_forward()


def head(x, spec):
    l1, l2, act = spec
    link = BceLink() if (HEAD_BCE and _BCE_HANDOFF[0] > 0 and torch.is_grad_enabled()) else None
    y = _Head.apply(x, l1.weight, l1.bias, l2.weight, l2.bias, act, link)
    if link is not None:
        y._sgg_bce_link = link
    return y


class ClipAdam:

    MAX_TENSORS = 48

    def __init__(self, params, lr, betas=(0.9, 0.999), eps=1e-8):
        self.params = [p for p in params]
        self.opt = torch.optim.Adam(self.params, lr=lr, betas=betas, eps=eps, capturable=True)
        self._ws = None

    def _state(self, p):
        st = self.opt.state[p]
        if "exp_avg" not in st:
            st["step"] = torch.zeros((), dtype=torch.float32, device=p.device)
            st["exp_avg"] = torch.zeros_like(p, memory_format=torch.preserve_format)
            st["exp_avg_sq"] = torch.zeros_like(p, memory_format=torch.preserve_format)
        elif not torch.is_tensor(st["step"]) or st["step"].device != p.device or st["step"].dtype != torch.float32:
            st["step"] = torch.as_tensor(float(st["step"]), dtype=torch.float32).to(p.device)
        return st

    @property
    def param_groups(self):
        return self.opt.param_groups

    def state_dict(self):
        return self.opt.state_dict()

    def load_state_dict(self, sd):
        self.opt.load_state_dict(sd)
        for p in self.params:
            if self.opt.state.get(p):
                self._state(p)

    def zero_grad(self, set_to_none=True):
        self.opt.zero_grad(set_to_none=set_to_none)

    def step(self, max_norm=0.0):
        lib = _lib()
        grp = self.opt.param_groups[0]
        act = [p for p in self.params if p.grad is not None]
        if max_norm > 0:
            self._launch(lib, act, grp, max_norm)
            return
        for i in range(0, len(act), self.MAX_TENSORS):
            self._launch(lib, act[i:i + self.MAX_TENSORS], grp, 0.0)

    def _launch(self, lib, act, grp, max_norm):
        import ctypes
        if len(act) > self.MAX_TENSORS:
            raise N.NativeError("ClipAdam: %d tensors with gradients, the fused step takes <= %d (clipping needs "
                              "them in one call)" % (len(act), self.MAX_TENSORS))
        for p in act:
            for t in (p, p.grad):
                if t.dtype != torch.float32 or not t.is_contiguous() or not t.is_cuda:
                    raise N.NativeError("ClipAdam: parameters and grads must be contiguous fp32 device tensors")
        n = len(act)
        st = [self._state(p) for p in act]
        for p in act:
            _EPOCH[p.data_ptr()] = _EPOCH.get(p.data_ptr(), 0) + 1
        arr = lambda xs: (ctypes.c_void_p * n)(*[x.data_ptr() for x in xs])
        numel = (ctypes.c_longlong * n)(*[p.numel() for p in act])
        total = sum(p.numel() for p in act)
        parts = lib.sgg_adam_parts(total)
        if self._ws is None or self._ws.numel() < parts:
            self._ws = torch.zeros(parts, device=act[0].device, dtype=torch.float32)
        b1, b2 = grp["betas"]
        N.check(lib.sgg_adam_step(arr(act), arr([p.grad for p in act]), arr([s["exp_avg"] for s in st]),
                                  arr([s["exp_avg_sq"] for s in st]), numel, n, float(grp["lr"]), float(b1),
                                  float(b2), float(grp["eps"]), float(max_norm), arr([s["step"] for s in st]),
                                  N.ptr(self._ws), self._ws.numel() * 4, N.stream_ptr()), "sgg_adam_step")


class OwnershipError(N.NativeError):
    """A re-issuable launch holds a raw device pointer (inside a ctypes
    descriptor) to memory it does not keep alive."""


def _storage_span(obj):
    s = obj.untyped_storage() if isinstance(obj, torch.Tensor) else obj
    b = s.data_ptr()
    return (b, b + s.nbytes())


def _walk_held(obj, spans, descs, seen, depth=0):
    import ctypes
    if obj is None or isinstance(obj, (int, float, str, bytes, bool)) or depth > 6 or id(obj) in seen:
        return
    seen.add(id(obj))
    if isinstance(obj, (torch.Tensor, torch.UntypedStorage)):
        sp = _storage_span(obj)
        if sp is not None:
            spans.append(sp)
        return
    if isinstance(obj, (ctypes.Structure, ctypes.Array)):
        descs.append(obj)
        for v in getattr(obj, "__dict__", {}).values():
            _walk_held(v, spans, descs, seen, depth + 1)
        return
    if isinstance(obj, (list, tuple, set, frozenset)):
        for v in obj:
            _walk_held(v, spans, descs, seen, depth + 1)
        return
    if isinstance(obj, dict):
        for v in obj.values():
            _walk_held(v, spans, descs, seen, depth + 1)
        return
    if isinstance(obj, functools.partial):
        for v in (obj.func, obj.args, obj.keywords):
            _walk_held(v, spans, descs, seen, depth + 1)
        return
    code = getattr(obj, "__code__", None)
    if code is not None:
        for c in obj.__closure__ or ():
            try:
                _walk_held(c.cell_contents, spans, descs, seen, depth + 1)
            except ValueError:
                pass
        _walk_held(obj.__defaults__, spans, descs, seen, depth + 1)
        _walk_held(obj.__kwdefaults__, spans, descs, seen, depth + 1)
        return
    if hasattr(obj, "__self__") and hasattr(obj, "__func__"):
        _walk_held(obj.__self__, spans, descs, seen, depth + 1)
        return
    d = getattr(obj, "__dict__", None)
    if d is not None and not isinstance(obj, (type, torch.nn.Module)):
        _walk_held(d, spans, descs, seen, depth + 1)


def _desc_pointers(desc, path="", out=None):
    import ctypes
    out = [] if out is None else out
    if isinstance(desc, ctypes.Array):
        for i in range(len(desc)):
            v = desc[i]
            if isinstance(v, (ctypes.Structure, ctypes.Array)):
                _desc_pointers(v, "%s[%d]" % (path, i), out)
            elif desc._type_ is ctypes.c_void_p and v:
                out.append(("%s[%d]" % (path, i), v))
        return out
    for fname, ftype in desc._fields_:
        v = getattr(desc, fname)
        if isinstance(v, (ctypes.Structure, ctypes.Array)):
            _desc_pointers(v, path + "." + fname, out)
        elif ftype is ctypes.c_void_p and v:
            out.append((path + "." + fname, v))
    return out


# ... 34 lines not shown
        gc.collect()
        gc.freeze()
    try:
        yield
    finally:
        if own:
            gc.unfreeze()


class LaunchTimer:

    def __init__(self):
        self.active = False
        self.rec = []

    def start(self):
        self.active, self.rec = True, []

    def stop(self):
        self.active = False
        torch.cuda.synchronize()
        out, self.rec = self.rec, []
        return out

    def add(self, name, key, flop, nbytes, relaunch):
        if self.active:
            check_ownership(relaunch, name)
            self.rec.append((name, (name,) + tuple(key), float(flop), float(nbytes), relaunch))

    @staticmethod
    def replay(records, reps=20):
        with capture_guard():
            return LaunchTimer._replay(records, reps)

    @staticmethod
    def _replay(records, reps):
        res = {}
        cur = torch.cuda.current_stream()
        for name, key, fl, nb, fn in records:
            if key in res:
                res[key]["launches"] += 1
                continue
            side = private_stream("timer")
            side.wait_stream(cur)
            graph = torch.cuda.CUDAGraph()
            try:
                with torch.cuda.stream(side):
                    fn()
                    graph.capture_begin(capture_error_mode=capture_error_mode())
                    for _ in range(reps):
                        fn()
                    graph.capture_end()
            except RuntimeError:
                graph = None
            cur.wait_stream(side)
            e0, e1 = torch.cuda.Event(enable_timing=True), torch.cuda.Event(enable_timing=True)
            e0.record()
            if graph is not None:
                graph.replay()
            else:
                for _ in range(reps):
                    fn()
            e1.record()
            e1.synchronize()
            res[key] = dict(name=name, launches=1, flop=fl, bytes=nb, ms=e0.elapsed_time(e1) / reps)
            del graph
        return res


timer = LaunchTimer()


def _pool_flops(scenes, bn):
    import numpy as np
    sz = np.diff(scenes.host_off).astype(np.float64)
    return float((sz * sz).sum()) * 512.0 * (4 + 2 * bn)


def _pool_kname(bn, gpw, nchunks, bf16, dev, max_n=None, max_rows=None):
    if bf16:
        g = 4 if gpw >= 4 and bn <= 48 else (2 if gpw >= 2 else 1)
        if max_n is not None and max_n >= 32 and os.environ.get("SGG_POOL_JB") != "0":
            gj = "*" if max_rows is None else (4 if max_rows > 16 else (2 if max_rows > 8 else 1))
            return "sgg::pool_fwd_bf16_jb_kernel<%d, %s>" % (bn, gj)
        return "sgg::pool_fwd_bf16_kernel<%d, %d>" % (bn, g)
    if gpw <= 2 and 32 <= bn <= 48 and os.environ.get("SGG_POOL_X3", "1")[:1] != "0":
        return "sgg::pool_fwd_x3_kernel<%d, %d>" % (bn, gpw)
    small = gpw <= 2 and nchunks <= 4 * torch.cuda.get_device_properties(dev).multi_processor_count
    return "sgg::" + ("pool_fwd_v_kernel<%d, %d>" % (bn, gpw) if small else "pool_fwd_kernel<%d, %d, 2>" % (bn, gpw))


def _pool_wbytes(bn):
    return 4.0 * (1024 + bn * 512 + bn)


class PoolRider:

    def __init__(self):
        self.held = None
        self.done = False
        self.carried = False

    def hold(self, batch, keep, weights, bn, bf16, gpw, nchunks, work, launch):
        self.held = (batch, keep, weights, bn, bf16, gpw, nchunks, work, launch)

    def fits(self, weights, bn, bf16, gpw, wide=False):
        if self.held is None or wide:
            return False
        _, _, wh, bnh, bfh, gph, _, _, _ = self.held
        return bnh == bn and bfh == bf16 and gph == gpw and all(a is b for a, b in zip(wh, weights))

    def carry(self, batch, keep, nchunks, work):
        a, keep_a, (A, W2, b2), bn, bf16, gpw, nch_a, work_a, _ = self.held
        self.held = None
        self.done = self.carried = True
        lib = _lib()
        b = batch

        def pl(k=(keep_a, keep, A, W2, b2)):
            N.check(lib.sgg_pool_fwd2(N.ctypes.byref(a), N.ctypes.byref(b), N.ptr(A), N.ptr(W2), N.ptr(b2), bn,
                                      int(bf16), N.stream_ptr()), "sgg_pool_fwd2")
        S2, B2 = work_a[0] + work[0], work_a[1] + work[1]
        return pl, (None, S2, B2, work_a[2] + work[2], work_a[3] + work[3], nch_a + nchunks)

    def flush(self):
        if self.held is not None:
            _, _, (A, W2, b2), bn, bf16, gpw, nch, work, launch = self.held
            self.held = None
            launch()
            if timer.active:
                timer.add(_pool_kname(bn, gpw, nch, bf16, A.device), work[:2], work[2], work[3] + _pool_wbytes(bn),
                          launch)
        self.done = True


_PRIDER = [None]


def pool_pair():
    return _scoped(_PRIDER, PoolRider())


def pool_is_wide(scenes):
    from .scene import SGG_POOL_MAX_PEDS, SGG_POOL_WIDE_MAX_PEDS
    if scenes.max_n > SGG_POOL_WIDE_MAX_PEDS:
        raise ValueError("social pooling: a scene of %d pedestrians exceeds the bound of %d per scene "
                         "(SGG_POOL_WIDE_MAX_PEDS)" % (scenes.max_n, SGG_POOL_WIDE_MAX_PEDS))
    return scenes.max_n > SGG_POOL_MAX_PEDS


class _Pool(torch.autograd.Function):

    @staticmethod
    def forward(ctx, h, pos, W1, We, be, b1, W2, b2, scenes, link=None, U=None, pdh=None):
        lib = _lib()
        ctx.link = link
        ctx.pdh = pdh
        wide = pool_is_wide(scenes)
        h = _rows(h, "h")
        pos = _req(pos, "pos").contiguous()
        B, Hd = h.shape
        E = We.shape[0]
        bn = W2.shape[0]
        assert pos.shape == (B, 2) and scenes.B == B, (pos.shape, B, scenes.B)
        assert W1.shape == (512, E + Hd), (W1.shape, E, Hd)
        W1 = W1.contiguous()
        W2 = W2.contiguous()
        b2 = b2.contiguous()
        A, c = fold_fwd(W1[:, :E], We, be, b1)
        if U is None:
            U = xw_raw(h, W1[:, E:], c, trans_w=True)
        else:
            assert U.shape == (B, 512) and U.is_contiguous()
        out = torch.empty(B, bn, device=h.device, dtype=torch.float32)
        am = torch.empty(B, bn, device=h.device, dtype=torch.int32)
        bf16 = _PRECISION == "bf16" and not wide
        plan = scenes.pool_plan(bn, wide=True) if wide else scenes.pool_plan(bn, bf16=bf16)
        chunks, nchunks, max_rows, gpw = plan[:4]
        ncd = plan[4] if len(plan) > 4 else None
        if bf16 and ncd is not None:
            gpw = 4

        if wide:
            def launch():
                N.check(lib.sgg_pool_fwd_wide(N.ptr(U), N.ptr(pos), N.ptr(A), N.ptr(W2), N.ptr(b2),
                                              N.ptr(scenes.scene_off), N.ptr(chunks), nchunks, max_rows, gpw, B, bn,
                                              scenes.max_n, N.ptr(out), N.ptr(am), N.stream_ptr()),
                        "sgg_pool_fwd_wide")
            kname = lambda nch: "sgg::pool_fwd_wide_kernel<%d, %d>" % (bn, gpw)
        else:
            fwd = lib.sgg_pool_fwd_bf16 if bf16 else lib.sgg_pool_fwd

            def launch():
                N.check(fwd(N.ptr(U), N.ptr(pos), N.ptr(A), N.ptr(W2), N.ptr(b2), N.ptr(scenes.scene_off),
                            N.ptr(chunks), nchunks, max_rows, gpw, B, bn, scenes.max_n, N.ptr(out),
                            N.ptr(am), N.ptr(ncd), N.stream_ptr()), "sgg_pool_fwd")
            kname = lambda nch: _pool_kname(bn, gpw, nch, bf16, h.device, scenes.max_n, max_rows)
        nb = 4.0 * (B * 512 + 2 * B) + 8.0 * B * bn
        work = (scenes.S, B, _pool_flops(scenes, bn), nb)
        rider = _PRIDER[0]
        if rider is not None and not wide and not rider.done and rider.held is None:
            batch = N.PoolBatch(N.ptr(U), N.ptr(pos), N.ptr(scenes.scene_off), N.ptr(chunks), nchunks, max_rows,
                                gpw, B, scenes.max_n, N.ptr(out), N.ptr(am), N.ptr(ncd))
            rider.hold(batch, (U, pos, scenes.scene_off, chunks, out, am, ncd), (A, W2, b2), bn, bf16, gpw,
                       nchunks, work, launch)
        elif rider is not None and rider.fits((A, W2, b2), bn, bf16, gpw, wide=wide):
            batch = N.PoolBatch(N.ptr(U), N.ptr(pos), N.ptr(scenes.scene_off), N.ptr(chunks), nchunks, max_rows,
                                gpw, B, scenes.max_n, N.ptr(out), N.ptr(am), N.ptr(ncd))
            pl, (name, S2, B2, fl2, nb2, nch2) = rider.carry(batch, (U, pos, scenes.scene_off, chunks, out, am, ncd),
                                                             nchunks, work)
            pl()
            if timer.active:
                timer.add(kname(nch2), (S2, B2, "pair"), fl2, nb2 + _pool_wbytes(bn), pl)
        else:
            if rider is not None:
                rider.flush()
            launch()
            if timer.active:
                timer.add(kname(nchunks), (scenes.S, B), work[2], nb + _pool_wbytes(bn), launch)
        ctx.scenes = scenes
        ctx.E = E
        ctx.save_for_backward(h, pos, W1, We, be, A, W2, U, out, am)
        ctx.mark_non_differentiable(am)
        ctx.set_materialize_grads(False)
        return out, am

    @staticmethod
    def backward(ctx, dout, _dam):
        lib = _lib()
        h, pos, W1, We, be, A, W2, U, out, am = ctx.saved_tensors
        sc, E = ctx.scenes, ctx.E
        B, bn = out.shape
        dout = dout.contiguous()
        need = ctx.needs_input_grad
        wgrad = any(need[2:8])
        P = bn * 512 + 1024 + bn
        dU = torch.empty(B, 512, device=h.device, dtype=torch.float32)
        wide = pool_is_wide(sc)
        rows = lib.sgg_pool_bwd_wide_grid(sc.S, sc.max_n) if wide else lib.sgg_pool_bwd_grid(sc.S)
        part = torch.empty(rows, P, device=h.device, dtype=torch.float32) if wgrad else None
        def launch():
            if wide:
                N.check(lib.sgg_pool_bwd_wide(N.ptr(U), N.ptr(pos), N.ptr(A), N.ptr(W2), N.ptr(out), N.ptr(am),
                                              N.ptr(dout), N.ptr(sc.scene_off), sc.S, B, bn, sc.max_n, N.ptr(dU),
                                              N.ptr(part), N.stream_ptr()), "sgg_pool_bwd_wide")
                return
            N.check(lib.sgg_pool_bwd(N.ptr(U), N.ptr(pos), N.ptr(A), N.ptr(W2), N.ptr(out), N.ptr(am), N.ptr(dout),
                                     N.ptr(sc.scene_off), sc.S, B, bn, sc.max_n, N.ptr(dU), N.ptr(part),
                                     N.stream_ptr()), "sgg_pool_bwd")
        launch()
        if timer.active:
            nb = 8.0 * B * 512 + 12.0 * B * bn + 4.0 * 512 * (2 + bn) + (4.0 * part.numel() if wgrad else 0.0)
            jq = max(1, min(8, 256 // sc.S)) if sc.S >= 1 else 1
            stage = (sc.max_n + jq - 1) // jq + 1 <= 16
            name = "sgg::pool_bwd_wide_kernel<%d, %s>" % (bn, "true" if wgrad else "false") if wide else \
                "sgg::pool_bwd_kernel<%d, %s, %s>" % (bn, "true" if wgrad else "false", "true" if stage else "false")
            timer.add(name, (sc.S, B), 8.0 * B * bn * 512, nb, launch)
        dh = None
        H = h.shape[1]
        dual = need[0] and wgrad and DUAL_POOL_BWD and H <= 64
        hand = ctx.pdh is not None and need[0] and not wide and (dual or not wgrad)
        if need[0]:
            base = ctx.link.take() if ctx.link is not None else None
            if hand:
                dh = base if base is not None else torch.empty(B, H, device=h.device, dtype=torch.float32)
                ride = wgrad and _DEFER[0] > 0
                ws, splits = None, 0
                if ride:
                    splits = lib.sgg_xtw_splits(B, H, 512)
                    ws = torch.empty(splits * (H * 512 + 512), device=h.device, dtype=torch.float32)
                ctx.pdh.put(dU, W1[:, E:], base, h, ws, splits, dh)
            elif dual:
                dh = base if base is not None else torch.empty(B, H, device=h.device, dtype=torch.float32)
                splits = lib.sgg_xtw_splits(B, H, 512)
                ws = torch.empty(splits * (H * 512 + 512), device=h.device, dtype=torch.float32)
                W1h = W1[:, E:]
                acc = int(base is not None)

                def launch2():
                    N.check(lib.sgg_pool_dh_dw(N.ptr(dU), 512, N.ptr(W1h), W1h.stride(0), N.ptr(dh), dh.stride(0),
                                               acc, N.ptr(h), h.stride(0), B, H, N.ptr(ws), ws.numel() * 4,
                                               N.stream_ptr()), "sgg_pool_dh_dw")
                launch2()
                if timer.active:
                    mt = 4 if H >= 64 else (H + 15) // 16
                    timer.add("sgg::xw_xtw_kernel<%d>" % mt, (B, H), 4.0 * B * 512 * H,
                              4.0 * (2 * B * 512 + 512 * H + 2 * B * H) + 4.0 * ws.numel(), launch2)
            else:
                dh = xw_raw(dU, W1[:, E:], None, trans_w=False, prec="fp32", out=base, act=0 if base is None else 2)
        if not wgrad:
            return dh, None, None, None, None, None, None, None, None, None, None, None
        rows = part.shape[0]
        if (not dual and not hand) or (hand and ws is None):
            ws, splits = xtw_partial(h, dU, colsum=True)
        dW1 = torch.empty_like(W1)
        dW2 = torch.empty(bn, 512, device=h.device, dtype=torch.float32)
        db2 = torch.empty(bn, device=h.device, dtype=torch.float32)
        dc = torch.empty(512, device=h.device, dtype=torch.float32)
        gf = GradFinish()
        gf.rowsum(part, rows, P, 0, bn * 512, dW2)
        gf.rowsum(part, rows, P, bn * 512 + 1024, bn, db2)
        gf.xtw_sums(ws, splits, H, 512, dW1[:, E:], trans_c=True, colsum=dc)
        _, dWe, dbe = gf.fold(W1[:, :E], We, be, part, rows, P, bn * 512, ws[splits * H * 512:], splits, 512, 0,
                              dW=dW1[:, :E])
        gf.run()
        return dh, None, dW1, dWe, dbe, dc, dW2, db2, None, None, None, None


class Handoff:

    def __init__(self):
        self.pending = None

    def put(self, *args):
        self.pending = args

    def take(self):
        p, self.pending = self.pending, None
        return p


class CopiesLink:

    def __init__(self):
        self.pending = None

    def put(self, base, copies, cstride, ld):
        self.pending = (base, copies, cstride, ld)

    def take(self):
        p, self.pending = self.pending, None
        return p


class GradLink:

    def __init__(self):
        self.grad = None

    def put(self, g):
        assert self.grad is None, "GradLink: gradient already pending"
        self.grad = g.contiguous()

    def take(self):
        g, self.grad = self.grad, None
        return g


class PoolDhSlot:

    def __init__(self):
        self.pending = None

    def put(self, *args):
        assert self.pending is None, "PoolDhSlot: a source is already pending"
        self.pending = args
        _PDH_OPEN.append(self)

    def take(self):
        p, self.pending = self.pending, None
        if p is not None:
            _PDH_OPEN.remove(self)
        return p


_PDH_OPEN = []


def _pooldh_standalone(src):
    dU, W1h, base, h, ws, splits, buf = src
    B, H = buf.shape
    if ws is not None:
        N.check(_lib().sgg_pool_dh_dw(N.ptr(dU), 512, N.ptr(W1h), W1h.stride(0), N.ptr(buf), buf.stride(0),
                                      int(base is not None), N.ptr(h), h.stride(0), B, H, N.ptr(ws), ws.numel() * 4,
                                      N.stream_ptr()), "sgg_pool_dh_dw")
    else:
        xw_raw(dU, W1h, None, trans_w=False, prec="fp32", out=buf, act=0 if base is None else 2)


def pooldh_check():
    if not _PDH_OPEN:
        return
    n = len(_PDH_OPEN)
    for slot in list(_PDH_OPEN):
        _pooldh_standalone(slot.take())
    raise RuntimeError("social pooling: %d backward(s) handed dh = dU W1h to an encoder backward that did not run "
                       "(SGG_POOL_DH_IN_LSTM=0 restores the stand-alone launches)" % n)


def social_pool(h, pos, W1, We, be, b1, W2, b2, scenes, link=None, U=None, dh_in_lstm=False):
    slot = None
    if dh_in_lstm and POOL_DH_IN_LSTM and U is not None and torch.is_grad_enabled():
        slot = getattr(U, "_sgg_pdh", None)
        if slot is not None and (pool_is_wide(scenes)
                                 or not _lib().sgg_lstm_bwd_pooldh_pays(h.numel() // h.shape[-1], h.shape[-1])):
            slot = None
    out, _ = _Pool.apply(h, pos, W1, We, be, b1, W2, b2, scenes, link, U, slot)
    return out


def pool_u_spec(pool):
    l1, E = pool.mlp_pre_pool[0], pool.embedding_dim
    _, c = fold_fwd(l1.weight[:, :E], pool.spatial_embedding.weight, pool.spatial_embedding.bias, l1.bias)
    return l1.weight[:, E:], c


def gat_wide_nodes(max_seg):
    from .scene import SGG_GAT_MAX_NODES, SGG_GAT_WIDE_MAX_NODES
    if max_seg > SGG_GAT_WIDE_MAX_NODES:
        raise ValueError("graph attention: a segment of %d nodes exceeds the bound of %d per segment "
                         "(SGG_GAT_WIDE_MAX_NODES)" % (max_seg, SGG_GAT_WIDE_MAX_NODES))
    return max_seg > SGG_GAT_MAX_NODES


def gat_is_wide(graph):
    return gat_wide_nodes(graph.max_seg)


def _gat_fwd_wide(wh, heads, a_src, a_dst, lda, bias, labels, seg_off, nseg, F, alpha, mode, epi, max_seg, hp, y):
    lib = _lib()
    n, HF = wh.shape
    work = torch.empty(int(lib.sgg_gat_wide_work_floats(n, nseg, heads, F, max_seg)), device=wh.device,
                       dtype=torch.float32)

    def launch():
        N.check(lib.sgg_gat_fwd_wide(N.ptr(wh), heads, N.ptr(a_src), N.ptr(a_dst), lda, N.ptr(bias), N.ptr(labels),
                                     N.ptr(seg_off), nseg, n, F, alpha, mode, epi, max_seg, N.ptr(hp), N.ptr(y), HF,
                                     N.ptr(work), N.stream_ptr()), "sgg_gat_fwd_wide")
    launch()
    if timer.active and n > 0:
        timer.add("sgg::gat_wide_scores_kernel+gat_fwd_wide_kernel", (n, HF, heads, max_seg),
                  2.0 * n * max_seg * HF, 4.0 * n * HF * (3 if epi else 2), launch)
    return work


def _gat_bwd_wide(wh, heads, a_src, a_dst, lda, labels, seg_off, nseg, F, alpha, mode, epi, max_seg, hp, y, dy, dWh,
                  ds, dt, da_s, da_d, dbias, work):
    lib = _lib()
    n, HF = wh.shape

    def launch():
        N.check(lib.sgg_gat_bwd_wide(N.ptr(wh), heads, N.ptr(a_src), N.ptr(a_dst), lda, N.ptr(labels), N.ptr(seg_off),
                                     nseg, n, F, alpha, mode, epi, max_seg, N.ptr(hp), N.ptr(y), N.ptr(dy), HF,
                                     N.ptr(dWh), N.ptr(ds), N.ptr(dt), N.ptr(da_s), N.ptr(da_d), N.ptr(dbias),
                                     N.ptr(work), N.stream_ptr()), "sgg_gat_bwd_wide")
    launch()
    if timer.active and n > 0:
        timer.add("sgg::gat_bwd_wide_rows_kernel+gat_bwd_wide_cols_kernel", (n, HF, heads, max_seg),
                  6.0 * n * max_seg * HF, 4.0 * n * HF * (4 if epi else 3), launch)


class _GatAttn(torch.autograd.Function):
    @staticmethod
    def forward(ctx, wh, a, bias, labels, seg_off, nseg, max_seg, alpha, mode, epi, heads):
        lib = _lib()
        wh = _req(wh, "wh").contiguous()
        n, HF = wh.shape
        F = HF // heads
        ctx.a_shape = a.shape
        a = a.contiguous().view(-1)
        if bias is not None:
            bias = bias.contiguous()
        y = torch.empty(n, HF, device=wh.device, dtype=torch.float32)
        hp = torch.empty(n, HF, device=wh.device, dtype=torch.float32) if epi else None
        work = None
        if gat_wide_nodes(max_seg):
            work = _gat_fwd_wide(wh, heads, a, a[F:], 2 * F, bias, labels, seg_off, nseg, F, float(alpha), mode, epi,
                                 max_seg, hp, y)
        else:
            N.check(lib.sgg_gat_fwd(N.ptr(wh), heads, N.ptr(a), N.ptr(bias), N.ptr(labels), N.ptr(seg_off), nseg, n, F,
                                    float(alpha), mode, epi, max_seg, N.ptr(hp), N.ptr(y), HF, N.stream_ptr()),
                    "sgg_gat_fwd")
        ctx.meta = (labels, seg_off, nseg, max_seg, float(alpha), mode, epi, heads, bias is not None)
        ctx.save_for_backward(wh, a, hp, y, work)
        return y

    @staticmethod
    def backward(ctx, dy):
        lib = _lib()
        wh, a, hp, y, work = ctx.saved_tensors
        labels, seg_off, nseg, max_seg, alpha, mode, epi, heads, has_bias = ctx.meta
        n, HF = wh.shape
        F = HF // heads
        dy = dy.contiguous()
        dWh = torch.empty(n, HF, device=wh.device, dtype=torch.float32)
        ds = torch.empty(n, heads, device=wh.device, dtype=torch.float32)
        dt = torch.empty(n, heads, device=wh.device, dtype=torch.float32)
        if work is not None:
            _gat_bwd_wide(wh, heads, a, a[F:], 2 * F, labels, seg_off, nseg, F, alpha, mode, epi, max_seg, hp, y, dy,
                          dWh, ds, dt, None, None, None, work)
        else:
            N.check(lib.sgg_gat_bwd(N.ptr(wh), heads, N.ptr(a), N.ptr(labels), N.ptr(seg_off), nseg, n, F, alpha, mode,
                                    epi, max_seg, N.ptr(hp), N.ptr(y), N.ptr(dy), HF, N.ptr(dWh), N.ptr(ds), N.ptr(dt),
                                    N.stream_ptr()), "sgg_gat_bwd")
        if not ctx.needs_input_grad[1] and not has_bias:
            return dWh, None, None, None, None, None, None, None, None, None, None
        dsdt = torch.cat([ds, dt], 1)
        if heads == 1:
            da = xtw(wh, dsdt).t().reshape(ctx.a_shape)
        else:
            C = xtw(wh, dsdt).view(heads, F, 2, heads)
            hh = torch.arange(heads, device=wh.device)
            da = C[hh, :, :, hh].permute(0, 2, 1).reshape(heads, 2 * F)
        dbias = None
        if has_bias:
            dpre = dy if epi == 0 else dy * torch.where(hp > 0, torch.ones_like(hp), torch.exp(hp))
            dbias = dpre.view(n, heads, F).double().sum((0, 1)).float()
        return dWh, da, dbias, None, None, None, None, None, None, None, None


class _GatAttnEx(torch.autograd.Function):

    @staticmethod
    def forward(ctx, wh, a_src, a_dst, bias, labels, seg_off, nseg, max_seg, alpha, mode, epi, heads):
        lib = _lib()
        wh = _req(wh, "wh").contiguous()
        n, HF = wh.shape
        F = HF // heads
        a_src, a_dst = a_src.contiguous(), a_dst.contiguous()
        if a_src.numel() != heads * F or a_dst.numel() != heads * F:
            raise ValueError("a_src / a_dst must hold heads x F = %d values" % (heads * F))
        if bias is not None:
            bias = bias.contiguous()
        y = torch.empty(n, HF, device=wh.device, dtype=torch.float32)
        hp = torch.empty(n, HF, device=wh.device, dtype=torch.float32) if epi else None
        work = None
        if gat_wide_nodes(max_seg):
            work = _gat_fwd_wide(wh, heads, a_src, a_dst, F, bias, labels, seg_off, nseg, F, float(alpha), mode, epi,
                                 max_seg, hp, y)
        else:
            N.check(lib.sgg_gat_fwd_ex(N.ptr(wh), heads, N.ptr(a_src), N.ptr(a_dst), N.ptr(bias), N.ptr(labels),
                                       N.ptr(seg_off), nseg, n, F, float(alpha), mode, epi, max_seg, N.ptr(hp),
                                       N.ptr(y), HF, N.stream_ptr()), "sgg_gat_fwd_ex")
        ctx.meta = (labels, seg_off, nseg, max_seg, float(alpha), mode, epi, heads, bias is not None, F)
        ctx.save_for_backward(wh, a_src, a_dst, hp, y, work)
        return y

    @staticmethod
    def backward(ctx, dy):
        lib = _lib()
        wh, a_src, a_dst, hp, y, work = ctx.saved_tensors
        labels, seg_off, nseg, max_seg, alpha, mode, epi, heads, has_bias, F = ctx.meta
        n, HF = wh.shape
        dy = dy.contiguous()
        dWh = torch.empty(n, HF, device=wh.device, dtype=torch.float32)
        da_s = torch.empty_like(a_src)
        da_d = torch.empty_like(a_dst)
        dbias = torch.empty(F, device=wh.device, dtype=torch.float32) if has_bias else None
        if work is not None:
            _gat_bwd_wide(wh, heads, a_src, a_dst, F, labels, seg_off, nseg, F, alpha, mode, epi, max_seg, hp, y, dy,
# ... 1585 lines not shown
```

### group-gan-gcn-gat_amd/sgan/train_step.py

```python
import contextlib
import collections
import functools
import os
import random
import time

import numpy as np
import torch
import torch.distributed as dist

from . import kernels as K
from .models import get_noise
from .scene import SceneIndex


PAIR = os.environ.get("SGG_PAIR", "1") != "0"
DEC_PAIR = os.environ.get("SGG_DEC_PAIR", "1") != "0"


class TrainArgs:

    def __init__(self, **kw):
        self.obs_len = 8
        self.pred_len = 12
        self.best_k = 20
        self.l2_loss_weight = 1.0
        self.clipping_threshold_g = 2.0
        self.clipping_threshold_d = 0.0
        self.g_learning_rate = 1e-4
        self.d_learning_rate = 1e-3
        self.__dict__.update(kw)


def _sse_of(sc):
    return torch.from_numpy(np.stack([sc.host_off[:-1], sc.host_off[1:]], 1))


def _valid(sc):
    nv = getattr(sc, "nvalid", None)
    return {"nvalid": nv} if nv is not None else {}


class DataParallel:

    def __init__(self, group=None, exercise=False, capture=None, transport=None):
        self.on = dist.is_available() and dist.is_initialized()
        self.group = group
        self.world = dist.get_world_size(group) if self.on else 1
        self.rank = dist.get_rank(group) if self.on else 0
        self.exercise = bool(exercise) and self.on
        if transport is None:
            transport = os.environ.get("SGG_DP_TRANSPORT") or (
                "rccl" if self.on and "nccl" in str(dist.get_backend(group)) else "pg")
        if transport not in ("rccl", "pg"):
            raise ValueError("DataParallel: transport %r (rccl | pg)" % (transport,))
        self.transport = transport
        if capture is None:
            capture = transport == "rccl" and os.environ.get("SGG_CAPTURE_COLLECTIVE", "1") != "0"
        if capture and transport != "rccl":
            raise ValueError("DataParallel: only the rccl transport's all-reduce can be captured in a graph")
        self.capture = bool(capture) and self.on
        self.cut = None

    @property
    def rccl(self):
        if self.transport != "rccl" or not self.collective:
            return None
        from .rccl import comm_for
        return comm_for(self.group)

    def prepare(self):
        self.rccl

    @property
    def collective(self):
        return self.on and (self.world > 1 or self.exercise)

    @property
    def segmented(self):
        return self.collective and not self.capture

    def shard(self, S_global):
        if S_global < self.world:
            raise ValueError("scene-sharded DP needs >= %d scenes (one per rank), got %d: the reference loader "
                             "keeps a short last batch (loader.py:22-27); drop it or run it on fewer ranks"
                             % (self.world, S_global))
        per, rem = divmod(S_global, self.world)
        s0 = self.rank * per + min(self.rank, rem)
        return s0, s0 + per + (1 if self.rank < rem else 0)

    def allreduce_(self, tensors):
        if not self.collective or not tensors:
            return
        if self.cut is not None:
            self.cut(tensors)
            return
        flat = torch.cat([t.reshape(-1) for t in tensors])
        if self.transport == "rccl":
            self.rccl.allreduce_sum_(flat)
        else:
            dist.all_reduce(flat, op=dist.ReduceOp.SUM, group=self.group)
        views = flat.split([t.numel() for t in tensors])
        torch._foreach_copy_(tensors, [v.view_as(t) for v, t in zip(views, tensors)])


class StepInputs:

    def __init__(self, z_d, z_g, y):
        self.z_d, self.z_g, self.y = z_d, z_g, y


class KernelOps:
    traj_cat = staticmethod(K.traj_cat)
    l2_select = staticmethod(K.l2_select)
    l2_loss = staticmethod(K.l2_loss)
    bce_pair = staticmethod(K.bce_pair)
    bce_pair_total = staticmethod(K.bce_pair_total)
    split2 = staticmethod(K.split2)
    prefold = staticmethod(K.prefold)
    one = staticmethod(lambda device: K.const(1.0, device))
    optimizer = staticmethod(lambda params, lr: K.ClipAdam(params, lr=lr))
    handoff = staticmethod(K.bce_handoff)
    defer_finish = staticmethod(K.defer_grad_finish)
    shared_prefix = staticmethod(K.shared_prefix)
    traj_ahead = staticmethod(K.traj_ahead)
    decoder_pair = staticmethod(K.decoder_pair)
    glue_ride = staticmethod(K.glue_ride)
    eager_losses = staticmethod(K.eager_losses)


class GanTrainer:
    def __init__(self, G, D, args=None, dp=None, selective_backward=True, capturable=False, bce_pair=None, ops=None):
        self.G, self.D = G, D
        self.ops = ops or KernelOps()
        self._bce_override = bce_pair
        self.bce_pair = bce_pair or self.ops.bce_pair
        self.args = args or TrainArgs()
        self.dp = dp or DataParallel()
        self.selective_backward = selective_backward
        bn = [n for n, m in list(G.named_modules()) + list(D.named_modules()) if isinstance(m, torch.nn.BatchNorm1d)]
        if bn:
            raise NotImplementedError("GanTrainer: BatchNorm layers (%s) are not supported (train.py's batch_norm=0 "
                                      "default); drive the modules with the reference's own step functions" % bn[:3])
        self.g_params = list(G.parameters())
        self.d_params = list(D.parameters())
        self.opt_g = self.ops.optimizer(self.g_params, self.args.g_learning_rate)
        self.opt_d = self.ops.optimizer(self.d_params, self.args.d_learning_rate)

    def _noise(self, S_global, s0, s1):
        G = self.G
        if not G.noise_dim:
            return None
        if G.noise_mix_type != "global":
            raise NotImplementedError("GanTrainer shards scenes; per-ped noise ('ped' mix) is not sharded yet")
        z = get_noise((S_global,) + tuple(G.noise_dim), G.noise_type)
        return z[s0:s1]

    def _finish(self, params, opt, loss_terms, clip):
        K.pooldh_check()
        K.grad_flush()
        grads = [p.grad for p in params if p.grad is not None]
        if self.dp.collective:
            vals = torch.stack([t.detach().reshape(()) for t in loss_terms])
            self.dp.allreduce_(grads + [vals])
        else:
            vals = [t.detach().reshape(()) for t in loss_terms]
        opt.step(max_norm=clip)
        return vals

    def _prefix(self, obs_rel, copies):
        sp = getattr(self.ops, "shared_prefix", None)
        if sp is None or getattr(self.D, "encoder", None) is None or os.environ.get("SGG_NO_SHARED_PREFIX"):
            return contextlib.nullcontext()
        return sp(self.D, obs_rel, self.args.obs_len + self.args.pred_len, copies)

    def _traj_ahead(self, head, T1, ncol, col0=0, b=None, pos0=None):
        ta = getattr(self.ops, "traj_ahead", None)
        if ta is None:
            return contextlib.nullcontext()
        return ta(head, T1, ncol, col0, b, pos0)

    def _scope(self):
        st = contextlib.ExitStack()
        st.enter_context(getattr(self.ops, "handoff", contextlib.nullcontext)())
        if not self._grad_observed():
            st.enter_context(getattr(self.ops, "defer_finish", contextlib.nullcontext)())
        st.enter_context(getattr(self.ops, "glue_ride", contextlib.nullcontext)())
        return st

    def _grad_observed(self):
        for p in self.g_params + self.d_params:
            if getattr(p, "_backward_hooks", None) or getattr(p, "_post_accumulate_grad_hooks", None) \
                    or p.retains_grad:
                return True
        return False

    def d_step(self, batch, sc, S_global=None, B_global=None, shard=(0, None), inputs=None, pair=None):
        with self._scope():
            return self._d_step(batch, sc, S_global, B_global, shard, inputs, pair)

    def _pairs(self, sc, sc_g):
        G = self.G
        return (PAIR and self.selective_backward and self.args.best_k > 1 and self.args.l2_loss_weight > 0
                and hasattr(G, "context_pair") and G.pair_ok(sc, sc_g))

    def _d_step(self, batch, sc, S_global, B_global, shard, inputs, pair=None):
        a = self.args
        G = self.G
        (obs, pred_gt, obs_rel, pred_gt_rel, _ov, _pv, obs_g, _pg, _nl, _lm, sse) = batch
        g_kw = (S_global, B_global)
        S_global = S_global or sc.S
        B_global = B_global or sc.B
        s0 = shard[0]
        z = inputs.z_d if inputs is not None else self._noise(S_global, s0, s0 + sc.S)
        prefold = getattr(self.ops, "prefold", None)
        if prefold is not None and hasattr(G, "fold_specs") and hasattr(self.D, "fold_specs") \
                and G.num_layers == 1 and self.D.encoder.num_layers == 1:
            prefold(G.fold_specs() + self.D.fold_specs())
        pre = None
        dpair = getattr(self.ops, "decoder_pair", None)
        dpair = dpair() if (pair is not None and DEC_PAIR and dpair is not None) else contextlib.nullcontext()
        with self._prefix(obs_rel, 2):
            with dpair:
                with self._traj_ahead(obs_rel, pred_gt_rel.shape[0], sc.B, 0, pred_gt_rel, obs[0]):
                    if pair is not None:
                        bg, scg = pair
                        ctx_d, ctx_g = G.context_pair((obs, obs_rel, sse, obs_g, sc),
                                                      (bg[0], bg[2], bg[10], bg[6], scg))
                        with torch.no_grad():
                            fake_rel = G.decode(ctx_d, obs, obs_rel, sse, user_noise=z, scenes=sc)
                    else:
                        with torch.no_grad():
                            fake_rel = G(obs, obs_rel, sse, obs_g, user_noise=z, scenes=sc)
                    traj_rel, start = self.ops.traj_cat(obs_rel, fake_rel, pred_gt_rel, obs[0])
                if pair is not None:
                    self._no_shared = True
                    try:
                        pre = self._g_prefix(bg, scg, g_kw[0], g_kw[1], shard, inputs, ctx=ctx_g)
                    finally:
                        self._no_shared = False
            sc2 = sc.repeat(2)
            scores = self.D(start, traj_rel, _sse_of(sc2), scenes=sc2)
        if inputs is not None:
            y_real = inputs.y[0]
        else:
            y_real = random.uniform(0.7, 1.2)
            random.uniform(0, 0.3)
        loss = self.bce_pair(scores, sc.B, 0.0, y_real, sc.B / B_global, **_valid(sc))
        self.opt_d.zero_grad(set_to_none=True)
        torch.autograd.backward(loss, grad_tensors=self.ops.one(loss.device))
        vals = self._finish(self.d_params, self.opt_d, [loss], a.clipping_threshold_d)
        out = {"D_data_loss": vals[0], "D_total_loss": vals[0]}
        return out if pair is None else (out, pre)

    def g_step(self, batch, sc, S_global=None, B_global=None, shard=(0, None), inputs=None):
        with self._scope():
            return self._g_step(batch, sc, S_global, B_global, shard, inputs)

    def _g_step(self, batch, sc, S_global, B_global, shard, inputs):
        return self._g_rest(self._g_prefix(batch, sc, S_global, B_global, shard, inputs))

    def g_prefix(self, batch, sc, S_global=None, B_global=None, shard=(0, None), inputs=None, shared=False):
        if shared:
            return self._g_prefix(batch, sc, S_global, B_global, shard, inputs)
        self._no_shared = True
        try:
            return self._g_prefix(batch, sc, S_global, B_global, shard, inputs)
        finally:
            self._no_shared = False

    def g_rest(self, pre):
        with self._scope():
            return self._g_rest(pre)

    def _g_prefix(self, batch, sc, S_global, B_global, shard, inputs, ctx=None):
        a = self.args
        G, ops = self.G, self.ops
        (obs, pred_gt, obs_rel, pred_gt_rel, _ov, _pv, obs_g, _pg, _nl, loss_mask, sse) = batch
        S_global = S_global or sc.S
        B_global = B_global or sc.B
        s0 = shard[0]
        S, B, k = sc.S, sc.B, a.best_k
        mask = loss_mask[:, a.obs_len:]
        if inputs is not None:
            z_all = inputs.z_g
        else:
            zs = [self._noise(S_global, s0, s0 + S) for _ in range(k)]
            z_all = torch.stack(zs, 0) if zs[0] is not None else None
        use_l2 = a.l2_loss_weight > 0
        pfx = None if getattr(self, "_no_shared", False) else self._prefix(obs_rel, 1)
        if pfx is not None:
            pfx.__enter__()
        try:
            if ctx is None:
                ctx = G.context(obs, obs_rel, sse, obs_g, scenes=sc)
            best = None
            if self.selective_backward and k > 1 and use_l2:
                with torch.no_grad():
                    pred_all = G.decode(ctx.detach(), obs, obs_rel, sse, user_noise=z_all, scenes=sc, copies=k,
                                        noise_index=(None, 0))
                    best = ops.l2_select(pred_all, pred_gt_rel, mask, sc, k)
        except BaseException:
            if pfx is not None:
                pfx.__exit__(None, None, None)
            raise
        return dict(batch=batch, sc=sc, S_global=S_global, B_global=B_global, z_all=z_all, ctx=ctx, best=best,
                    pfx=pfx, mask=mask, inputs=inputs)

    def _g_rest(self, pre):
        a = self.args
        G, D, ops = self.G, self.D, self.ops
        batch, sc, B_global, z_all, ctx, pfx, mask, inputs = (pre[n] for n in (
# ... 525 lines not shown
```

### include/sgg.h

```cpp
#ifndef SGG_H
#define SGG_H

#include <stdint.h>
#include <stddef.h>

#ifdef __cplusplus
extern "C" {
#endif

#define SGG_E_ARG (-1)

int sgg_version(void);
const char* sgg_last_error(void);
const char* sgg_source_hash(void);

#define SGG_POOL_MAX_PEDS 64
#define SGG_POOL_WIDE_MAX_PEDS 1024
#define SGG_GAT_MAX_NODES 128
#define SGG_GAT_WIDE_MAX_NODES 1024

int sgg_xw(const float* X, int ldx, const float* Xmask, int ldm, const float* W, int ldw, int trans_w,
           const float* bias, float* Y, int ldy, int M, int K, int N, int act, void* stream);

int sgg_xw_bf16(const float* X, int ldx, const float* Xmask, int ldm, const float* W, int ldw, int trans_w,
                const float* bias, float* Y, int ldy, int M, int K, int N, int act, void* stream);

int sgg_pool_plan(const int32_t* host_scene_off, int S, int bn, int target_chunks, int max_gpw,
                  int32_t* host_chunks, int cap, int* max_rows, int* gpw);
int sgg_pool_fwd(const float* U, const float* pos, const float* A, const float* W2,
                 const float* b2, const int32_t* scene_off, const int32_t* chunks, int nchunks,
                 int max_rows, int gpw, int B, int bn, int max_n, float* out, int32_t* argmax,
                 const int32_t* nchunks_dev, void* stream);

int sgg_pool_plan_bf16(const int32_t* host_scene_off, int S, int bn, int target_chunks, int32_t* host_chunks,
                       int cap, int* max_rows, int* gpw);
int sgg_pool_fwd_bf16(const float* U, const float* pos, const float* A, const float* W2,
                      const float* b2, const int32_t* scene_off, const int32_t* chunks, int nchunks,
                      int max_rows, int gpw, int B, int bn, int max_n, float* out, int32_t* argmax,
                      const int32_t* nchunks_dev, void* stream);

typedef struct SggPoolBatch {
  const float* U;
  const float* pos;
  const int32_t* scene_off;
  const int32_t* chunks;
  int nchunks;
  int max_rows;
  int gpw;
  int B;
  int max_n;
  float* out;
  int32_t* argmax;
  const int32_t* nchunks_dev;
} SggPoolBatch;
int sgg_pool_fwd2(const SggPoolBatch* a, const SggPoolBatch* b, const float* A, const float* W2, const float* b2,
                  int bn, int bf16, void* stream);

int sgg_pool_dh_dw(const float* dU, int ldu, const float* W, int ldw, float* dh, int ldh, int accumulate,
                   const float* h, int ldx, int B, int H, float* ws, size_t ws_bytes, void* stream);

int sgg_pool_bwd_grid(int S);
int sgg_pool_bwd(const float* U, const float* pos, const float* A, const float* W2,
                 const float* out, const int32_t* argmax, const float* dout,
                 const int32_t* scene_off, int S, int B, int bn, int max_n,
                 float* dU, float* part, void* stream);

int sgg_pool_plan_wide(const int32_t* host_scene_off, int S, int bn, int target_chunks, int32_t* host_chunks,
                       int cap, int* max_rows, int* gpw);
int sgg_pool_fwd_wide(const float* U, const float* pos, const float* A, const float* W2,
                      const float* b2, const int32_t* scene_off, const int32_t* chunks, int nchunks,
                      int max_rows, int gpw, int B, int bn, int max_n, float* out, int32_t* argmax,
                      void* stream);
int sgg_pool_bwd_wide_grid(int S, int max_n);
int sgg_pool_bwd_wide(const float* U, const float* pos, const float* A, const float* W2,
                      const float* out, const int32_t* argmax, const float* dout,
                      const int32_t* scene_off, int S, int B, int bn, int max_n,
                      float* dU, float* part, void* stream);

int sgg_gat_fwd(const float* Wh, int heads, const float* a, const float* bias, const float* labels,
                const int32_t* seg_off, int nseg, int n, int F, float alpha, int mask_mode,
                int epilogue, int max_seg, float* hp, float* y, int ldy, void* stream);

int sgg_gat_bwd(const float* Wh, int heads, const float* a, const float* labels, const int32_t* seg_off,
                int nseg, int n, int F, float alpha, int mask_mode, int epilogue, int max_seg,
                const float* hp, const float* y, const float* dy, int lddy,
                float* dWh, float* ds, float* dt, void* stream);

int sgg_gat_fwd_ex(const float* Wh, int heads, const float* a_src, const float* a_dst, const float* bias,
                   const float* labels, const int32_t* seg_off, int nseg, int n, int F, float alpha, int mask_mode,
                   int epilogue, int max_seg, float* hp, float* y, int ldy, void* stream);

size_t sgg_gat_bwd_ex_work_bytes(int nseg, int heads, int F);
int sgg_gat_bwd_ex(const float* Wh, int heads, const float* a_src, const float* a_dst, const float* labels,
                   const int32_t* seg_off, int nseg, int n, int F, float alpha, int mask_mode, int epilogue,
                   int max_seg, const float* hp, const float* y, const float* dy, int lddy, float* dWh,
                   float* da_src, float* da_dst, float* dbias, void* work, void* stream);

size_t sgg_gat_wide_work_floats(int n, int nseg, int heads, int F, int max_seg);
int sgg_gat_fwd_wide(const float* Wh, int heads, const float* a_src, const float* a_dst, int lda,
                     const float* bias, const float* labels, const int32_t* seg_off, int nseg, int n, int F,
                     float alpha, int mask_mode, int epilogue, int max_seg, float* hp, float* y, int ldy,
                     float* work, void* stream);
int sgg_gat_bwd_wide(const float* Wh, int heads, const float* a_src, const float* a_dst, int lda,
                     const float* labels, const int32_t* seg_off, int nseg, int n, int F, float alpha,
                     int mask_mode, int epilogue, int max_seg, const float* hp, const float* y,
                     const float* dy, int lddy, float* dWh, float* ds, float* dt, float* da_src,
                     float* da_dst, float* dbias, float* work, void* stream);

size_t sgg_gat_layer_lds_bytes(int K, int F, int max_seg);
int sgg_gat_layer_fwd(const float* x1, int ld1, int K1, const float* x2, int ld2, int K2, const float* w,
                      const float* a_src, const float* a_dst, const float* bias, const int32_t* seg_off, int nseg,
                      int n, int heads, int F, float alpha, float eps, int epilogue, int max_seg, int bf16,
                      float* xn, float* rstd, float* wh, float* hp, float* y, int ldy, void* stream);

typedef struct SggGatLayerSet {
  const float* x1;
  int ld1, K1;
  const float* x2;
  int ld2, K2;
  const int32_t* seg_off;
  int nseg, n, max_seg;
  float *xn, *rstd, *wh, *hp, *y;
  int ldy;
} SggGatLayerSet;
int sgg_gat_layer_fwd2(const SggGatLayerSet* a, const SggGatLayerSet* b, const float* w, const float* a_src,
                       const float* a_dst, const float* bias, int heads, int F, float alpha, float eps,
                       int epilogue, int bf16, void* stream);

int sgg_seg_norm_fwd(const float* x, int ldx, int F, const int32_t* seg_off, int nseg, float eps,
                     float* y, int ldy, float* rstd, void* stream);

int sgg_seg_norm_bwd(const float* y, int ldy, const float* dy, int lddy, int F, const int32_t* seg_off,
                     int nseg, const float* rstd, float* dx, int lddx, void* stream);

size_t sgg_group_index_ws(int S, int B);
int sgg_group_index(const float* labels, const int32_t* scene_off, int S, int B, int max_n,
                    int32_t* ped_gid, int32_t* ped_scene, int32_t* group_off,
                    int32_t* group_scene, int32_t* group_count, void* workspace, void* stream);

int sgg_seg_reduce(const float* x, int ldx, int F, const int32_t* seg_of_row,
                   const float* row_scale, const int32_t* range_off, const int32_t* seg_range,
                   const int32_t* nseg_dev, int nseg_cap, int mean, float* out, int ldo,
                   void* stream);

int sgg_seg_gather(const float* src, int lds, int F, const int32_t* seg_of_row,
                   const float* row_scale, const int32_t* nrow_dev, int n, float* out, int ldo,
                   void* stream);

int sgg_xtw_splits(int R, int M, int N);
int sgg_xtw(const float* X, int ldx, const float* Y, int ldy, const float* Ymask, int ldm, int R, int M, int N,
            float* C, int ldc, int trans_c, float* colsum, float* ws, size_t ws_bytes, void* stream);
int sgg_xtw_partial(const float* X, int ldx, const float* Y, int ldy, const float* Ymask, int ldm, int R, int M,
                    int N, int colsum, float* ws, size_t ws_bytes, void* stream);

#define SGG_RED_MAX 24
#define SGG_FOLDB_MAX 6
typedef struct {
  const float* src;
  int rows;
  int ld;
  int col0;
  int cols;
  float* out;
  int map;
  int N;
  int ldo;
  int trans;
} SggRed;
typedef struct {
  const float* W;
  int ldw;
  int R;
  int E;
  const float* We;
  const float* be;
  const float* dA_src;
  int dA_rows;
  int dA_ld;
  int dA_col0;
  const float* db_src;
  int db_rows;
  int db_ld;
  int db_col0;
  float* dW;
  int lddw;
  float* dWe;
  float* dbe;
  float* dbias_copy;
} SggFoldBwd;
int sgg_grad_finish(const SggRed* reds, int nred, const SggFoldBwd* folds, int nfold, float* scratch,
                    size_t scratch_bytes, void* stream);

#define SGG_LOSSJOB_MAX 2
typedef struct {
  const float* term;
  int S;
  float* loss;
} SggL2Job;
typedef struct {
  const float* x;
  int n;
  int split;
  const float* ya;
  const float* yb;
  float w;
  float* loss;
  const float* addend;
  float* total;
  const int32_t* nvalid;
} SggBceJob;
int sgg_grad_finish_losses(const SggRed* reds, int nred, const SggFoldBwd* folds, int nfold, float* scratch,
                           size_t scratch_bytes, const SggL2Job* l2, int nl2, const SggBceJob* bce, int nbce,
                           void* stream);

int sgg_head_ok(int K, int N1);
int sgg_head_slab_cols(int K, int N1);
int sgg_head_fwd(const float* X, int ldx, int M, int K, int N1, const float* W1, const float* b1, const float* w2,
                 const float* b2, int act, float* hid, float* Y, void* stream);
// ... 282 lines not shown
```

Measured before the change: 146,400 scenes/s.

## Fuse the scoring head's forward and backward into the pooling backward kernel

Adds a pool_bwd_head_kernel that recomputes the discriminator scoring head (linear, ReLU, linear, BCE gradient) on the pooled rows inside the pooling backward, producing the head's input gradient directly in shared memory instead of reading dout from a separate head launch. Shared head device helpers move into a header so both files can use them. Python wiring uses a HeadSlot to defer the head's own launch to the pooling backward, with fallbacks and checks when the handoff does not happen. This removes a kernel launch and a global round trip of the head gradient, at the cost of extra shared memory, registers and synchronisation in the pooling kernel.

```diff
diff --git a/group-gan-gcn-gat_amd/csrc/head.hip b/group-gan-gcn-gat_amd/csrc/head.hip
--- a/group-gan-gcn-gat_amd/csrc/head.hip
+++ b/group-gan-gcn-gat_amd/csrc/head.hip
@@ -1,16 +1,8 @@
-#include "sgg_common.h"
+#include "head_body.h"
 
 namespace sgg {
 
 namespace {
-
-constexpr int kHeadRows = 64;
-
-__device__ __forceinline__ float bce_grad(float x, float y) {
-  const float e = expf(-fabsf(x));
-  const float sg = x > 0.f ? 1.f : (x < 0.f ? -1.f : 0.f);
-  return (x >= 0.f ? 1.f : 0.f) - y - sg * (e / (1.f + e));
-}
 
 template <int NT, int KT>
 __global__ void __launch_bounds__(256) head_fwd_kernel(const float* __restrict__ X, int ldx, int M,
@@ -73,73 +65,6 @@
     const int m = row0 + 4 * q + r;
     if (c16 == 0 && m < M) Y[m] = y;
   }
-}
-
-template <int NT, int KT, int DP>
-__device__ __forceinline__ void head_bwd_tail(const float* __restrict__ X, int ldx, int M, int rb,
-                                              const float (&dh)[kHeadRows][DP], const float (&hg)[kHeadRows][DP],
-                                              const float (&g2s)[kHeadRows], const float (&wb)[4 * NT][KT],
-                                              float* __restrict__ dX, int lddx, float* __restrict__ wslab) {
-  constexpr int N1 = 16 * NT, K = 16 * KT;
-  const int tid = threadIdx.x;
-  const int lane = tid & 63, wave = tid >> 6;
-  const int c16 = lane & 15, q = lane >> 4;
-  {
-    floatx4 acc[KT];
-#pragma unroll
-    for (int t = 0; t < KT; ++t) acc[t] = floatx4{0.f, 0.f, 0.f, 0.f};
-#pragma unroll
-    for (int s = 0; s < N1 / 4; ++s) {
-      const float a = dh[16 * wave + c16][4 * s + q];
-#pragma unroll
-      for (int t = 0; t < KT; ++t) acc[t] = __builtin_amdgcn_mfma_f32_16x16x4f32(a, wb[s][t], acc[t], 0, 0, 0);
-    }
-#pragma unroll
-    for (int t = 0; t < KT; ++t)
-#pragma unroll
-      for (int r = 0; r < 4; ++r) {
-        const int m = rb + 16 * wave + 4 * q + r;
-        if (m < M) dX[(size_t)m * lddx + 16 * t + c16] = acc[t][r];
-      }
-  }
-  if (!wslab) return;
-  float* row = wslab + (size_t)blockIdx.x * (N1 * K + 2 * N1 + 1);
-  for (int tile = wave; tile < NT * KT; tile += 4) {
-    const int mt = tile / KT, nt = tile - mt * KT;
-    floatx4 acc = floatx4{0.f, 0.f, 0.f, 0.f};
-    float xb[kHeadRows / 4];
-#pragma unroll
-    for (int s = 0; s < kHeadRows / 4; ++s)
-      xb[s] = X[(size_t)min(rb + 4 * s + q, M - 1) * ldx + 16 * nt + c16];
-#pragma unroll
-    for (int s = 0; s < kHeadRows / 4; ++s) {
-      const float a = dh[4 * s + q][16 * mt + c16];
-      acc = __builtin_amdgcn_mfma_f32_16x16x4f32(a, xb[s], acc, 0, 0, 0);
-    }
-#pragma unroll
-    for (int r = 0; r < 4; ++r) row[(size_t)(16 * mt + 4 * q + r) * K + 16 * nt + c16] = acc[r];
-  }
-  for (int n = tid; n < N1; n += 256) {
-    float s1 = 0.f, s2 = 0.f;
-    for (int r = 0; r < kHeadRows; ++r) {
-      s1 += dh[r][n];
-      s2 += hg[r][n];
-    }
-    row[N1 * K + n] = s1;
-    row[N1 * K + N1 + n] = s2;
-  }
-  if (tid == 0) {
-    float s = 0.f;
-    for (int r = 0; r < kHeadRows; ++r) s += g2s[r];
-    row[N1 * K + 2 * N1] = s;
-  }
-}
-
-__device__ __forceinline__ float bce_dy(float y, int m, int M, float gw, float ya, float yb, int split, int nv) {
-  const bool first = m < split;
-  const float cnt = first ? (float)min(split, nv) : (float)min(M - split, nv);
-  const bool live = first ? m < nv : m - split < nv;
-  return live ? (gw / cnt) * bce_grad(y, first ? ya : yb) : 0.f;
 }
 
 template <int NT, int KT>
diff --git a/group-gan-gcn-gat_amd/csrc/head_body.h b/group-gan-gcn-gat_amd/csrc/head_body.h
--- /dev/null
+++ b/group-gan-gcn-gat_amd/csrc/head_body.h
@@ -0,0 +1,200 @@
+#pragma once
+#include "sgg_common.h"
+
+namespace sgg {
+
+namespace {
+
+constexpr int kHeadRows = 64;
+
+__device__ __forceinline__ float bce_grad(float x, float y) {
+  const float e = expf(-fabsf(x));
+  const float sg = x > 0.f ? 1.f : (x < 0.f ? -1.f : 0.f);
+  return (x >= 0.f ? 1.f : 0.f) - y - sg * (e / (1.f + e));
+}
+
+template <int NT, int KT, int DP>
+__device__ __forceinline__ void head_bwd_tail(const float* __restrict__ X, int ldx, int M, int rb,
+                                              const float (&dh)[kHeadRows][DP], const float (&hg)[kHeadRows][DP],
+                                              const float (&g2s)[kHeadRows], const float (&wb)[4 * NT][KT],
+                                              float* __restrict__ dX, int lddx, float* __restrict__ wslab) {
+  constexpr int N1 = 16 * NT, K = 16 * KT;
+  const int tid = threadIdx.x;
+  const int lane = tid & 63, wave = tid >> 6;
+  const int c16 = lane & 15, q = lane >> 4;
+  {
+    floatx4 acc[KT];
+#pragma unroll
+    for (int t = 0; t < KT; ++t) acc[t] = floatx4{0.f, 0.f, 0.f, 0.f};
+#pragma unroll
+    for (int s = 0; s < N1 / 4; ++s) {
+      const float a = dh[16 * wave + c16][4 * s + q];
+#pragma unroll
+      for (int t = 0; t < KT; ++t) acc[t] = __builtin_amdgcn_mfma_f32_16x16x4f32(a, wb[s][t], acc[t], 0, 0, 0);
+    }
+#pragma unroll
+    for (int t = 0; t < KT; ++t)
+#pragma unroll
+      for (int r = 0; r < 4; ++r) {
+        const int m = rb + 16 * wave + 4 * q + r;
+        if (m < M) dX[(size_t)m * lddx + 16 * t + c16] = acc[t][r];
+      }
+  }
+  if (!wslab) return;
+  float* row = wslab + (size_t)blockIdx.x * (N1 * K + 2 * N1 + 1);
+  for (int tile = wave; tile < NT * KT; tile += 4) {
+    const int mt = tile / KT, nt = tile - mt * KT;
+    floatx4 acc = floatx4{0.f, 0.f, 0.f, 0.f};
+    float xb[kHeadRows / 4];
+#pragma unroll
+    for (int s = 0; s < kHeadRows / 4; ++s)
+      xb[s] = X[(size_t)min(rb + 4 * s + q, M - 1) * ldx + 16 * nt + c16];
+#pragma unroll
+    for (int s = 0; s < kHeadRows / 4; ++s) {
+      const float a = dh[4 * s + q][16 * mt + c16];
+      acc = __builtin_amdgcn_mfma_f32_16x16x4f32(a, xb[s], acc, 0, 0, 0);
+    }
+#pragma unroll
+    for (int r = 0; r < 4; ++r) row[(size_t)(16 * mt + 4 * q + r) * K + 16 * nt + c16] = acc[r];
+  }
+  for (int n = tid; n < N1; n += 256) {
+    float s1 = 0.f, s2 = 0.f;
+    for (int r = 0; r < kHeadRows; ++r) {
+      s1 += dh[r][n];
+      s2 += hg[r][n];
+    }
+    row[N1 * K + n] = s1;
+    row[N1 * K + N1 + n] = s2;
+  }
+  if (tid == 0) {
+    float s = 0.f;
+    for (int r = 0; r < kHeadRows; ++r) s += g2s[r];
+    row[N1 * K + 2 * N1] = s;
+  }
+}
+
+__device__ __forceinline__ float bce_dy(float y, int m, int M, float gw, float ya, float yb, int split, int nv) {
+  const bool first = m < split;
+  const float cnt = first ? (float)min(split, nv) : (float)min(M - split, nv);
+  const bool live = first ? m < nv : m - split < nv;
+  return live ? (gw / cnt) * bce_grad(y, first ? ya : yb) : 0.f;
+}
+
+template <int KT>
+struct HeadFwdJob {
+  float a[4 * KT], b[4 * KT], bc;
+};
+
+template <int KT>
+__device__ __forceinline__ void head_fwd_job_load(HeadFwdJob<KT>& j, const float* __restrict__ xr,
+                                                  const float* __restrict__ W1, const float* __restrict__ b1, int t) {
+  constexpr int K = 16 * KT;
+  const int lane = threadIdx.x & 63;
+  const int c16 = lane & 15, q = lane >> 4;
+  const float* wr = W1 + (size_t)(16 * t + c16) * K;
+#pragma unroll
+  for (int m = 0; m < KT; ++m) {
+    const float4 xv = *reinterpret_cast<const float4*>(xr + 16 * m + 4 * q);
+    const float4 wv = *reinterpret_cast<const float4*>(wr + 16 * m + 4 * q);
+    j.a[4 * m] = xv.x;
+    j.a[4 * m + 1] = xv.y;
+    j.a[4 * m + 2] = xv.z;
+    j.a[4 * m + 3] = xv.w;
+    j.b[4 * m] = wv.x;
+    j.b[4 * m + 1] = wv.y;
+    j.b[4 * m + 2] = wv.z;
+    j.b[4 * m + 3] = wv.w;
+  }
+  j.bc = b1[16 * t + c16];
+}
+
+template <int KT, int DP>
+__device__ __forceinline__ void head_fwd_job_run(const HeadFwdJob<KT>& j, int act, int lr0, int t, float (*hh)[DP]) {
+  const int lane = threadIdx.x & 63;
+  const int c16 = lane & 15, q = lane >> 4;
+  floatx4 acc = floatx4{0.f, 0.f, 0.f, 0.f};
+#pragma unroll
+  for (int s = 0; s < 4 * KT; ++s) acc = __builtin_amdgcn_mfma_f32_16x16x4f32(j.a[s], j.b[s], acc, 0, 0, 0);
+#pragma unroll
+  for (int r = 0; r < 4; ++r) {
+    float v = acc[r] + j.bc;
+    if (act & 1) v = v > 0.f ? v : 0.f;
+    hh[lr0 + 4 * q + r][16 * t + c16] = v;
+  }
+}
+
+template <int NT>
+struct HeadScoreOps {
+  float wc[NT], bb2, gw, ya, yb;
+  int nv;
+};
+
+template <int NT>
+__device__ __forceinline__ void head_score_load(HeadScoreOps<NT>& o, int M, const float* __restrict__ w2,
+                                                const float* __restrict__ b2, const float* __restrict__ bce_g,
+                                                const float* __restrict__ bce_ya, const float* __restrict__ bce_yb,
+                                                float bce_w, const int32_t* __restrict__ bce_nvalid) {
+  const int c16 = threadIdx.x & 15;
+#pragma unroll
+  for (int t = 0; t < NT; ++t) o.wc[t] = w2[16 * t + c16];
+  o.bb2 = b2[0];
+  o.gw = *bce_g * bce_w;
+  o.ya = *bce_ya;
+  o.yb = *bce_yb;
+  o.nv = bce_nvalid ? *bce_nvalid : M;
+}
+
+template <int NT, int DP>
+__device__ __forceinline__ void head_score_stage(const HeadScoreOps<NT>& o, int act, int lr0, int m0, int nrows, int M,
+                                                 int bce_split, float* __restrict__ Y, float (*hh)[DP]) {
+  const int lane = threadIdx.x & 63;
+  const int c16 = lane & 15, q = lane >> 4;
+  float h[NT][4];
+  float p[4] = {0.f, 0.f, 0.f, 0.f};
+#pragma unroll
+  for (int t = 0; t < NT; ++t)
+#pragma unroll
+    for (int r = 0; r < 4; ++r) {
+      const float v = hh[lr0 + 4 * q + r][16 * t + c16];
+      h[t][r] = v;
+      p[r] = fmaf(v, o.wc[t], p[r]);
+    }
+#pragma unroll
+  for (int r = 0; r < 4; ++r) {
+#pragma unroll
+    for (int x = 1; x < 16; x <<= 1) p[r] += __shfl_xor(p[r], x);
+    float y = p[r] + o.bb2;
+    if (act & 2) y = y > 0.f ? y : 0.f;
+    const int i = 4 * q + r, m = m0 + i;
+    const bool live = i < nrows;
+    if (Y && c16 == 0 && live) Y[m] = y;
+    const float dy = bce_dy(y, min(m, M - 1), M, o.gw, o.ya, o.yb, bce_split, o.nv);
+    const float g = (live && (!(act & 2) || y > 0.f)) ? dy : 0.f;
+#pragma unroll
+    for (int t = 0; t < NT; ++t) hh[lr0 + i][16 * t + c16] = (!(act & 1) || h[t][r] > 0.f) ? g * o.wc[t] : 0.f;
+  }
+}
+
+template <int NT, int KT>
+__device__ __forceinline__ void head_dx_job_load(float (&wb)[4 * NT], const float* __restrict__ W1, int t) {
+  constexpr int K = 16 * KT;
+  const int lane = threadIdx.x & 63;
+  const int c16 = lane & 15, q = lane >> 4;
+#pragma unroll
+  for (int s = 0; s < 4 * NT; ++s) wb[s] = W1[(size_t)(4 * s + q) * K + 16 * t + c16];
+}
+
+template <int NT, int DP>
+__device__ __forceinline__ floatx4 head_dx_job_run(const float (&wb)[4 * NT], const float (*dh)[DP], int lr0) {
+  const int lane = threadIdx.x & 63;
+  const int c16 = lane & 15, q = lane >> 4;
+  floatx4 acc = floatx4{0.f, 0.f, 0.f, 0.f};
+#pragma unroll
+  for (int s = 0; s < 4 * NT; ++s)
+    acc = __builtin_amdgcn_mfma_f32_16x16x4f32(dh[lr0 + c16][4 * s + q], wb[s], acc, 0, 0, 0);
+  return acc;
+}
+
+}
+
+}
diff --git a/group-gan-gcn-gat_amd/csrc/pool.hip b/group-gan-gcn-gat_amd/csrc/pool.hip
--- a/group-gan-gcn-gat_amd/csrc/pool.hip
+++ b/group-gan-gcn-gat_amd/csrc/pool.hip
@@ -3,6 +3,7 @@
 
 #include "sgg_common.h"
 #include "pool_common.h"
+#include "head_body.h"
 
 namespace sgg {
 
@@ -990,12 +991,13 @@
 
 constexpr int kBwdStageRows = 16;
 
-template <int BN, bool WGRAD, bool STAGE>
-__global__ void __launch_bounds__(512) pool_bwd_kernel(
-    const float* __restrict__ U, const float* __restrict__ pos, const float* __restrict__ A,
-    const float* __restrict__ W2 , const float* __restrict__ out,
-    const int32_t* __restrict__ argmax, const float* __restrict__ dout, const int32_t* __restrict__ scene_off,
-    int S, int jq, float* __restrict__ dU, float* __restrict__ part) {
+template <int BN, bool WGRAD, bool STAGE, int NT>
+__device__ __forceinline__ void pool_bwd_body(
+    const float* U, const float* pos, const float* A,
+    const float* W2 , const float* out,
+    const int32_t* argmax, const float* dout, const int32_t* scene_off,
+    int S, int jq, float* dU, float* part, const SggPoolHead& hp) {
+  constexpr bool HEAD = NT > 0;
   __shared__ unsigned long long msk[SGG_POOL_MAX_PEDS * BN];
   __shared__ float gs[SGG_POOL_MAX_PEDS * BN];
   __shared__ int jsel[SGG_POOL_MAX_PEDS * BN];
@@ -1021,16 +1023,72 @@
 #pragma unroll 4
       for (int r = 0; r < j1 - j0; ++r) Us[r * kHidden + k] = Ur[(size_t)r * kHidden];
     }
+    if constexpr (HEAD) {
+      static_assert(BN % 16 == 0, "the head's input width is a multiple of 16");
+      constexpr int KT = BN / 16, DP = 16 * NT + 4;
+      __shared__ float hd[SGG_POOL_MAX_PEDS][DP];
+      const int wave = __builtin_amdgcn_readfirstlane(k >> 6);
+      const int lane = k & 63, c16 = lane & 15, q4 = lane >> 4;
+      const int rt_n = (n + 15) >> 4, nf = rt_n * NT, nb = rt_n * KT;
+      HeadFwdJob<KT> fj;
+      float wb[4 * NT];
+      HeadScoreOps<NT> so;
+      auto fwd_load = [&](int job) {
+        const int rt = job / NT;
+        head_fwd_job_load<KT>(fj, out + (size_t)(o + min(16 * rt + c16, n - 1)) * BN, hp.W1, hp.b1, job - rt * NT);
+      };
+      auto dx_run = [&](int job) {
+        const int rt = job / KT, t = job - rt * KT;
+        const floatx4 acc = head_dx_job_run<NT, DP>(wb, hd, 16 * rt);
+#pragma unroll
+        for (int r = 0; r < 4; ++r) {
+          const int i = 16 * rt + 4 * q4 + r;
+          if (i < n) {
+            const int e = i * BN + 16 * t + c16;
+            gs[e] = gs[e] > 0.f ? acc[r] : 0.f;
+          }
+        }
+      };
+      if (wave < nf) fwd_load(wave);
+      if (wave < nb) head_dx_job_load<NT, KT>(wb, hp.W1, wave % KT);
+      if (wave < rt_n) head_score_load<NT>(so, hp.M, hp.w2, hp.b2, hp.g, hp.ya, hp.yb, hp.w, hp.nvalid);
 #pragma unroll 2
-    for (int e = k; e < ne; e += kHidden) {
-      const size_t ge = (size_t)o * BN + e;
-      const float ov = out[ge], dv = dout[ge];
-      const int av = argmax[ge];
-      gs[e] = ov > 0.f ? dv : 0.f;
-      jsel[e] = av - o;
-      msk[e] = 0ull;
-    }
-    for (int q = k; q < n; q += kHidden) ps[q] = make_float2(pos[2 * (o + q)], pos[2 * (o + q) + 1]);
+      for (int e = k; e < ne; e += kHidden) {
+        const size_t ge = (size_t)o * BN + e;
+        const float ov = out[ge];
+        const int av = argmax[ge];
+        gs[e] = ov;
+        jsel[e] = av - o;
+        msk[e] = 0ull;
+      }
+      for (int q = k; q < n; q += kHidden) ps[q] = make_float2(pos[2 * (o + q)], pos[2 * (o + q) + 1]);
+      if (wave < nf) head_fwd_job_run<KT, DP>(fj, hp.act, 16 * (wave / NT), wave % NT, hd);
+      if (wave + 8 < nf) {
+        fwd_load(wave + 8);
+        head_fwd_job_run<KT, DP>(fj, hp.act, 16 * ((wave + 8) / NT), (wave + 8) % NT, hd);
+      }
+      __syncthreads();
+      if (wave < rt_n)
+        head_score_stage<NT, DP>(so, hp.act, 16 * wave, o + 16 * wave, n - 16 * wave, hp.M, hp.split,
+                                 jp == 0 ? hp.Y : nullptr, hd);
+      __syncthreads();
+      if (wave < nb) dx_run(wave);
+      if (wave + 8 < nb) {
+        head_dx_job_load<NT, KT>(wb, hp.W1, (wave + 8) % KT);
+        dx_run(wave + 8);
+      }
+    } else {
+#pragma unroll 2
+      for (int e = k; e < ne; e += kHidden) {
+        const size_t ge = (size_t)o * BN + e;
+        const float ov = out[ge], dv = dout[ge];
+        const int av = argmax[ge];
+        gs[e] = ov > 0.f ? dv : 0.f;
+        jsel[e] = av - o;
+        msk[e] = 0ull;
+      }
+      for (int q = k; q < n; q += kHidden) ps[q] = make_float2(pos[2 * (o + q)], pos[2 * (o + q) + 1]);
+    }
     __syncthreads();
     for (int e = k; e < ne; e += kHidden) {
       if (gs[e] != 0.f) {
@@ -1103,6 +1161,24 @@
   }
 }
 
+template <int BN, bool WGRAD, bool STAGE>
+__global__ void __launch_bounds__(512) pool_bwd_kernel(
+    const float* __restrict__ U, const float* __restrict__ pos, const float* __restrict__ A,
+    const float* __restrict__ W2 , const float* __restrict__ out,
+    const int32_t* __restrict__ argmax, const float* __restrict__ dout, const int32_t* __restrict__ scene_off,
+    int S, int jq, float* __restrict__ dU, float* __restrict__ part) {
+  pool_bwd_body<BN, WGRAD, STAGE, 0>(U, pos, A, W2, out, argmax, dout, scene_off, S, jq, dU, part, SggPoolHead{});
+}
+
+template <int BN, bool WGRAD, bool STAGE, int NT>
+__global__ void __launch_bounds__(512) pool_bwd_head_kernel(
+    const float* __restrict__ U, const float* __restrict__ pos, const float* __restrict__ A,
+    const float* __restrict__ W2 , const float* __restrict__ out,
+    const int32_t* __restrict__ argmax, const int32_t* __restrict__ scene_off, int S, int jq,
+    float* __restrict__ dU, float* __restrict__ part, SggPoolHead hp) {
+  pool_bwd_body<BN, WGRAD, STAGE, NT>(U, pos, A, W2, out, argmax, nullptr, scene_off, S, jq, dU, part, hp);
+}
+
 template <int BN>
 static size_t pool_fwd_lds(int max_rows) {
   using C = PoolCfg<BN>;
@@ -1219,6 +1295,33 @@
   }
 #undef SGG_POOL_BWD
   SGG_RETURN_LAUNCH("sgg_pool_bwd");
+}
+
+template <int BN, int NT>
+static int launch_bwd_head(const float* U, const float* pos, const float* A, const float* W2, const float* out,
+                           const int32_t* am, const SggPoolHead& hp, const int32_t* off, int S, int max_n, float* dU,
+                           hipStream_t st) {
+  const int grid = sgg_pool_bwd_grid(S), jq = pool_bwd_jq(S);
+  const int rows = (max_n + jq - 1) / jq + 1;
+  const bool stage = rows <= kBwdStageRows;
+  const size_t lds = stage ? sizeof(float) * (size_t)rows * kHidden : 0;
+#define SGG_POOL_BWD_HEAD(SG)                                                                                      \
+  hipLaunchKernelGGL((pool_bwd_head_kernel<BN, false, SG, NT>), dim3(grid), dim3(512), lds, st, U, pos, A, W2, out, \
+                     am, off, S, jq, dU, nullptr, hp)
+  if (stage) SGG_POOL_BWD_HEAD(true); else SGG_POOL_BWD_HEAD(false);
+#undef SGG_POOL_BWD_HEAD
+  SGG_RETURN_LAUNCH("sgg_pool_bwd_head");
+}
+
+template <int BN>
+static int launch_bwd_head_n1(const float* U, const float* pos, const float* A, const float* W2, const float* out,
+                              const int32_t* am, const SggPoolHead& hp, const int32_t* off, int S, int max_n,
+                              float* dU, hipStream_t st) {
+  switch (hp.N1) {
+    case 16: return launch_bwd_head<BN, 1>(U, pos, A, W2, out, am, hp, off, S, max_n, dU, st);
+    case 32: return launch_bwd_head<BN, 2>(U, pos, A, W2, out, am, hp, off, S, max_n, dU, st);
+    default: return launch_bwd_head<BN, 4>(U, pos, A, W2, out, am, hp, off, S, max_n, dU, st);
+  }
 }
 
 }
@@ -1425,3 +1528,35 @@
     default: return launch_bwd<64>(U, pos, A, W2, out, argmax, dout, scene_off, S, max_n, dU, part, st);
   }
 }
+
+extern "C" int sgg_pool_bwd_head_ok(int bn, int N1) {
+  return (bn == 32 || bn == 48) && (N1 == 16 || N1 == 32 || N1 == 64);
+}
+
+extern "C" int sgg_pool_bwd_head_pays(int S, int max_n, int wgrad) {
+  return !wgrad && S >= 1 && S <= 256 && max_n >= 1 && max_n <= SGG_POOL_MAX_PEDS;
+}
+
+extern "C" int sgg_pool_bwd_head(const float* U, const float* pos, const float* A, const float* W2, const float* out,
+                                 const int32_t* argmax, const SggPoolHead* head, const int32_t* scene_off, int S,
+                                 int B, int bn, int max_n, float* dU, void* stream) {
+  SGG_CHECK_ARG(U && pos && A && W2 && out && argmax && head && scene_off && dU, "sgg_pool_bwd_head: null pointer");
+  SGG_CHECK_ARG(head->W1 && head->b1 && head->w2 && head->b2 && head->Y && head->g && head->ya && head->yb,
+                "sgg_pool_bwd_head: null pointer in the head's arguments");
+  SGG_CHECK_ARG(sgg_pool_bwd_head_ok(bn, head->N1) && head->K == bn,
+                "sgg_pool_bwd_head: bottleneck %d with a head of K=%d N1=%d not built (bn = K in {32, 48}, N1 in "
+                "{16, 32, 64})", bn, head->K, head->N1);
+  SGG_CHECK_ARG(head->act >= 0 && head->act <= 3, "sgg_pool_bwd_head: act %d outside [0, 3]", head->act);
+  SGG_CHECK_ARG(max_n >= 1 && max_n <= SGG_POOL_MAX_PEDS, "sgg_pool_bwd_head: max scene size %d outside [1, %d]",
+                max_n, SGG_POOL_MAX_PEDS);
+  SGG_CHECK_ARG(S >= 0 && B >= 0 && head->M == B, "sgg_pool_bwd_head: bad sizes (S=%d B=%d, the head's M=%d)", S, B,
+                head->M);
+  SGG_CHECK_ARG(head->split >= 0 && head->split <= head->M, "sgg_pool_bwd_head: BCE split %d outside [0, %d]",
+                head->split, head->M);
+  SGG_CHECK_ARG(((reinterpret_cast<uintptr_t>(out) | reinterpret_cast<uintptr_t>(head->W1)) & 15) == 0,
+                "sgg_pool_bwd_head: out and W1 must be 16-byte aligned");
+  hipStream_t st = (hipStream_t)stream;
+  if (S == 0) return 0;
+  if (bn == 32) return launch_bwd_head_n1<32>(U, pos, A, W2, out, argmax, *head, scene_off, S, max_n, dU, st);
+  return launch_bwd_head_n1<48>(U, pos, A, W2, out, argmax, *head, scene_off, S, max_n, dU, st);
+}
diff --git a/group-gan-gcn-gat_amd/sgan/_native.py b/group-gan-gcn-gat_amd/sgan/_native.py
--- a/group-gan-gcn-gat_amd/sgan/_native.py
+++ b/group-gan-gcn-gat_amd/sgan/_native.py
@@ -103,6 +103,11 @@
 class PoolBatch(ctypes.Structure):
     _fields_ = [("U", _p), ("pos", _p), ("scene_off", _p), ("chunks", _p), ("nchunks", _i), ("max_rows", _i),
                 ("gpw", _i), ("B", _i), ("max_n", _i), ("out", _p), ("argmax", _p), ("nchunks_dev", _p)]
+
+
+class PoolHead(ctypes.Structure):
+    _fields_ = [("W1", _p), ("b1", _p), ("w2", _p), ("b2", _p), ("act", _i), ("N1", _i), ("K", _i), ("Y", _p),
+                ("g", _p), ("ya", _p), ("yb", _p), ("split", _i), ("w", _f), ("nvalid", _p), ("M", _i)]
 
 
 class GatLayerSet(ctypes.Structure):
@@ -134,6 +139,9 @@
     "sgg_pool_bwd_grid": (_i, [_i]),
     "sgg_pool_dh_dw": (_i, [_p, _i, _p, _i, _p, _i, _i, _p, _i, _i, _i, _p, _sz, _p]),
     "sgg_pool_bwd": (_i, [_p, _p, _p, _p, _p, _p, _p, _p, _i, _i, _i, _i, _p, _p, _p]),
+    "sgg_pool_bwd_head_ok": (_i, [_i, _i]),
+    "sgg_pool_bwd_head_pays": (_i, [_i, _i, _i]),
+    "sgg_pool_bwd_head": (_i, [_p, _p, _p, _p, _p, _p, ctypes.POINTER(PoolHead), _p, _i, _i, _i, _i, _p, _p]),
     "sgg_pool_plan_wide": (_i, [_p, _i, _i, _i, _p, _i, _p, _p]),
     "sgg_pool_fwd_wide": (_i, [_p, _p, _p, _p, _p, _p, _p, _i, _i, _i, _i, _i, _i, _p, _p, _p]),
     "sgg_pool_bwd_wide_grid": (_i, [_i, _i]),
diff --git a/group-gan-gcn-gat_amd/sgan/kernels.py b/group-gan-gcn-gat_amd/sgan/kernels.py
--- a/group-gan-gcn-gat_amd/sgan/kernels.py
+++ b/group-gan-gcn-gat_amd/sgan/kernels.py
@@ -11,6 +11,7 @@
 GATENC_SAVE = os.environ.get("SGG_GATENC_SAVE", "1") != "0"
 DUAL_POOL_BWD = os.environ.get("SGG_DUAL_POOL_BWD", "1") != "0"
 POOL_DH_IN_LSTM = os.environ.get("SGG_POOL_DH_IN_LSTM", "1") != "0"
+HEAD_IN_POOL = os.environ.get("SGG_HEAD_IN_POOL", "1") != "0"
 
 
 DEBUG = os.environ.get("SGG_DEBUG", "0") == "1"
@@ -466,6 +467,7 @@
     def __init__(self):
         self.pending = None
         self.forward_held = None
+        self.head_slot = None
         self.fused = None
 
     def put(self, g, ya, yb, split, w, placeholder, nvalid=None):
@@ -480,6 +482,12 @@
         if held is None:
             return
         x, W1, b1, W2, b2, act, y, wgrad = held
+        slot = self.head_slot
+        if slot is not None:
+            if HEAD_IN_POOL and not wgrad and _loss_deferrable("bce"):
+                slot.hold(self, (x, W1, b1, W2, b2, act, y), (ya, yb, int(split), float(w), nvalid))
+                return
+            self.head_slot = None
         lib = _lib()
         M, Kd = x.shape
         N1 = W1.shape[0]
@@ -560,6 +568,15 @@
         N1 = W1.shape[0]
         link = ctx.bce_link
         pend = link.take() if link is not None else None
+        slot = link.head_slot if link is not None else None
+        if slot is not None and slot.held is not None:
+            if pend is None or dy.data_ptr() != pend[5].data_ptr():
+                slot.standalone(pend[0] if pend is not None else None)
+                raise N.NativeError("head inside the pooling backward: the scores have a consumer besides the BCE "
+                                    "loss (set SGG_HEAD_IN_POOL=0)")
+            dxp = torch.empty(M, Kd, device=x.device, dtype=torch.float32)
+            slot.put(pend[0].contiguous(), dxp)
+            return dxp, None, None, None, None, None, None
         if link is not None and link.forward_held is not None:
             link.flush_forward()
         fused, hid = None, ctx.hid
@@ -635,6 +652,11 @@
 def head(x, spec):
     l1, l2, act = spec
     link = BceLink() if (HEAD_BCE and _BCE_HANDOFF[0] > 0 and torch.is_grad_enabled()) else None
+    slot = getattr(x, "_sgg_head_slot", None)
+    if (slot is not None and link is not None and HEAD_FUSE and HEAD_IN_POOL and x.dim() == 2 and x.shape[0] > 0
+            and x.is_contiguous() and x.data_ptr() % 16 == 0
+            and _lib().sgg_pool_bwd_head_ok(l1.in_features, l1.out_features)):
+        link.head_slot = slot
     y = _Head.apply(x, l1.weight, l1.bias, l2.weight, l2.bias, act, link)
     if link is not None:
         y._sgg_bce_link = link
@@ -975,10 +997,13 @@
 class _Pool(torch.autograd.Function):
 
     @staticmethod
-    def forward(ctx, h, pos, W1, We, be, b1, W2, b2, scenes, link=None, U=None, pdh=None):
+    def forward(ctx, h, pos, W1, We, be, b1, W2, b2, scenes, link=None, U=None, pdh=None, hslot=None):
         lib = _lib()
         ctx.link = link
         ctx.pdh = pdh
+        ctx.hslot = hslot if (hslot is not None and not any(ctx.needs_input_grad[2:8])) else None
+        if hslot is not None and ctx.hslot is None:
+            hslot.armed = False
         wide = pool_is_wide(scenes)
         h = _rows(h, "h")
         pos = _req(pos, "pos").contiguous()
@@ -1062,7 +1087,22 @@
         wide = pool_is_wide(sc)
         rows = lib.sgg_pool_bwd_wide_grid(sc.S, sc.max_n) if wide else lib.sgg_pool_bwd_grid(sc.S)
         part = torch.empty(rows, P, device=h.device, dtype=torch.float32) if wgrad else None
+        hd = ctx.hslot.take() if ctx.hslot is not None else None
+        if hd is not None and (hd.dxp is None or dout.data_ptr() != hd.dxp.data_ptr()):
+            hd.standalone()
+            raise N.NativeError("head inside the pooling backward: the gradient of the pooled rows is not the "
+                                "head's alone (set SGG_HEAD_IN_POOL=0)")
+        if hd is not None:
+            hx, hW1, hb1, hW2, hb2, hact, hy = hd.head
+            hya, hyb, hsplit, hw, hnv = hd.bce
+            harg = N.PoolHead(N.ptr(hW1), N.ptr(hb1), N.ptr(hW2), N.ptr(hb2), hact, hW1.shape[0], hW1.shape[1],
+                              N.ptr(hy), N.ptr(hd.g), N.ptr(hya), N.ptr(hyb), hsplit, hw, N.ptr(hnv), B)
         def launch():
+            if hd is not None:
+                N.check(lib.sgg_pool_bwd_head(N.ptr(U), N.ptr(pos), N.ptr(A), N.ptr(W2), N.ptr(out), N.ptr(am),
+                                              N.ctypes.byref(harg), N.ptr(sc.scene_off), sc.S, B, bn, sc.max_n,
+                                              N.ptr(dU), N.stream_ptr()), "sgg_pool_bwd_head")
+                return
             if wide:
                 N.check(lib.sgg_pool_bwd_wide(N.ptr(U), N.ptr(pos), N.ptr(A), N.ptr(W2), N.ptr(out), N.ptr(am),
                                               N.ptr(dout), N.ptr(sc.scene_off), sc.S, B, bn, sc.max_n, N.ptr(dU),
@@ -1078,7 +1118,13 @@
             stage = (sc.max_n + jq - 1) // jq + 1 <= 16
             name = "sgg::pool_bwd_wide_kernel<%d, %s>" % (bn, "true" if wgrad else "false") if wide else \
                 "sgg::pool_bwd_kernel<%d, %s, %s>" % (bn, "true" if wgrad else "false", "true" if stage else "false")
-            timer.add(name, (sc.S, B), 8.0 * B * bn * 512, nb, launch)
+            fl = 8.0 * B * bn * 512
+            if hd is not None:
+                N1 = hd.head[1].shape[0]
+                name = "sgg::pool_bwd_head_kernel<%d, false, %s, %d>" % (bn, "true" if stage else "false", N1 // 16)
+                fl += jq * (2.0 * B * N1 * (bn + 1) + 2.0 * B * N1 * bn)
+                nb += 4.0 * (N1 * bn + 2 * N1 + 1 + B) - 4.0 * B * bn
+            timer.add(name, (sc.S, B), fl, nb, launch)
         dh = None
         H = h.shape[1]
         dual = need[0] and wgrad and DUAL_POOL_BWD and H <= 64
@@ -1112,7 +1158,7 @@
             else:
                 dh = xw_raw(dU, W1[:, E:], None, trans_w=False, prec="fp32", out=base, act=0 if base is None else 2)
         if not wgrad:
-            return dh, None, None, None, None, None, None, None, None, None, None, None
+            return dh, None, None, None, None, None, None, None, None, None, None, None, None
         rows = part.shape[0]
         if (not dual and not hand) or (hand and ws is None):
             ws, splits = xtw_partial(h, dU, colsum=True)
@@ -1127,7 +1173,7 @@
         _, dWe, dbe = gf.fold(W1[:, :E], We, be, part, rows, P, bn * 512, ws[splits * H * 512:], splits, 512, 0,
                               dW=dW1[:, :E])
         gf.run()
-        return dh, None, dW1, dWe, dbe, dc, dW2, db2, None, None, None, None
+        return dh, None, dW1, dWe, dbe, dc, dW2, db2, None, None, None, None, None
 
 
 class Handoff:
@@ -1211,6 +1257,55 @@
                        "(SGG_POOL_DH_IN_LSTM=0 restores the stand-alone launches)" % n)
 
 
+class HeadSlot:
+
+    def __init__(self):
+        self.armed = True
+        self.held = None
+        self.g = None
+        self.dxp = None
+
+    def hold(self, link, head, bce):
+        self.held = link
+        self.head, self.bce = head, bce
+        _HEAD_OPEN.append(self)
+
+    def put(self, g, dxp):
+        self.g, self.dxp = g, dxp
+
+    def take(self):
+        if self.held is None:
+            return None
+        self.held = None
+        _HEAD_OPEN.remove(self)
+        return self
+
+    def standalone(self, g=None):
+        if self.held is not None:
+            self.take()
+        x, W1, b1, W2, b2, act, y = self.head
+        ya, yb, split, w, nvalid = self.bce
+        g = self.g if self.g is not None else (g.contiguous() if g is not None else const(1.0, x.device))
+        M, Kd = x.shape
+        dx = self.dxp if self.dxp is not None else torch.empty(M, Kd, device=x.device, dtype=torch.float32)
+        N.check(_lib().sgg_head_fwdbwd(N.ptr(x), x.stride(0), M, Kd, W1.shape[0], N.ptr(W1), N.ptr(b1), N.ptr(W2),
+                                       N.ptr(b2), act, N.ptr(y), N.ptr(dx), dx.stride(0), None, N.ptr(g), N.ptr(ya),
+                                       N.ptr(yb), split, w, N.ptr(nvalid), N.stream_ptr()), "sgg_head_fwdbwd")
+
+
+_HEAD_OPEN = []
+
+
+def headpool_check():
+    if not _HEAD_OPEN:
+        return
+    n = len(_HEAD_OPEN)
+    for slot in list(_HEAD_OPEN):
+        slot.standalone()
+    raise RuntimeError("scoring head: %d head(s) left their launch to a pooling backward that did not run "
+                       "(SGG_HEAD_IN_POOL=0 restores the head's own launch)" % n)
+
+
 def social_pool(h, pos, W1, We, be, b1, W2, b2, scenes, link=None, U=None, dh_in_lstm=False):
     slot = None
     if dh_in_lstm and POOL_DH_IN_LSTM and U is not None and torch.is_grad_enabled():
@@ -1218,7 +1313,13 @@
         if slot is not None and (pool_is_wide(scenes)
                                  or not _lib().sgg_lstm_bwd_pooldh_pays(h.numel() // h.shape[-1], h.shape[-1])):
             slot = None
-    out, _ = _Pool.apply(h, pos, W1, We, be, b1, W2, b2, scenes, link, U, slot)
+    hslot = None
+    if (HEAD_IN_POOL and torch.is_grad_enabled() and _BCE_HANDOFF[0] > 0 and _DEFER[0] > 0
+            and not pool_is_wide(scenes) and _lib().sgg_pool_bwd_head_pays(scenes.S, scenes.max_n, 0)):
+        hslot = HeadSlot()
+    out, _ = _Pool.apply(h, pos, W1, We, be, b1, W2, b2, scenes, link, U, slot, hslot)
+    if hslot is not None and hslot.armed:
+        out._sgg_head_slot = hslot
     return out
 
 
diff --git a/group-gan-gcn-gat_amd/sgan/train_step.py b/group-gan-gcn-gat_amd/sgan/train_step.py
--- a/group-gan-gcn-gat_amd/sgan/train_step.py
+++ b/group-gan-gcn-gat_amd/sgan/train_step.py
@@ -158,6 +158,7 @@
 
     def _finish(self, params, opt, loss_terms, clip):
         K.pooldh_check()
+        K.headpool_check()
         K.grad_flush()
         grads = [p.grad for p in params if p.grad is not None]
         if self.dp.collective:
diff --git a/include/sgg.h b/include/sgg.h
--- a/include/sgg.h
+++ b/include/sgg.h
@@ -64,6 +64,28 @@
                  const float* out, const int32_t* argmax, const float* dout,
                  const int32_t* scene_off, int S, int B, int bn, int max_n,
                  float* dU, float* part, void* stream);
+
+typedef struct {
+  const float* W1;
+  const float* b1;
+  const float* w2;
+  const float* b2;
+  int act, N1, K;
+  float* Y;
+  const float* g;
+  const float* ya;
+  const float* yb;
+  int split;
+  float w;
+  const int32_t* nvalid;
+  int M;
+} SggPoolHead;
+int sgg_pool_bwd_head_ok(int bn, int N1);
+int sgg_pool_bwd_head_pays(int S, int max_n, int wgrad);
+int sgg_pool_bwd_head(const float* U, const float* pos, const float* A, const float* W2,
+                      const float* out, const int32_t* argmax, const SggPoolHead* head,
+                      const int32_t* scene_off, int S, int B, int bn, int max_n,
+                      float* dU, void* stream);
 
 int sgg_pool_plan_wide(const int32_t* host_scene_off, int S, int bn, int target_chunks, int32_t* host_chunks,
                        int cap, int* max_rows, int* gpw);
```

Measured after the change: 147,600 scenes/s, median of 6. No clear change (+0.9%).
